# huggingface/tokenizers

Hardware: AMD Instinct MI355X
Metric: GB input text/sec (whole node), GPT-2 BPE encode_batch (higher is better)
Workload: dtype u8->u32

## Files before the change

tokenizers_amd/csrc/capi/api_handle.cpp:

```cpp

#pragma GCC visibility push(default)
extern "C" {

const char* tkamd_version(void) { return "tokenizers_amd 0.1.0 (gfx950)"; }
const char* tkamd_last_error(void) { return g_last_error.c_str(); }

static std::unique_ptr<tkamd_tokenizer> make_tokenizer(const char* json, size_t json_len, int device, const tkamd_tokenizer* primary) {
    std::unique_ptr<tkamd_tokenizer> t(new tkamd_tokenizer());
    if (primary) { t->hm = primary->hm; t->n_direct = primary->n_direct; }
    else t->hm = HostModel::from_json(json, json_len);
    t->device = device;
    if (device >= 0) {
        check_not_forked();
        int n = 0;
        if (hipGetDeviceCount(&n) != hipSuccess || n == 0) throw HipError("no HIP device available (the HIP path has no CPU fallback)");
        if (device >= n) throw HipError("HIP device ordinal out of range");
        HIP_CHECK(hipSetDevice(device));
        note_hip_used();
        hipDeviceProp_t prop;
        HIP_CHECK(hipGetDeviceProperties(&prop, device));
        t->n_cu = prop.multiProcessorCount > 0 ? prop.multiProcessorCount : 256;
        if (const char* e = test_hook("TKAMD_Q16_DIV")) t->q16_div = (uint32_t)std::max(1, atoi(e));
        upload_tables(t.get());
        if (prepare_long_kernel() != 0) throw HipError("hipFuncSetAttribute(dynamic LDS) failed");
        if (!primary) verify_direct_words(t.get());
        build_shortw_table(t.get());
        build_hot_table(t.get());
        if (const char* e = test_hook("TKAMD_CLAIMS_PAUSE")) t->claims_pause_len = std::max(0, atoi(e));
        if (const char* e = test_hook("TKAMD_ADDED_SPEC")) t->added_spec_len = std::max(0, atoi(e));
        if (const char* e = test_hook("TKAMD_NFC_SPEC")) t->nfc_spec_len = std::max(0, atoi(e));
        t->cp_grid = compact_grid(t->n_cu);
        if (const char* e = test_hook("TKAMD_CP_GRID")) t->cp_grid = std::max(1, atoi(e));
        t->devices.push_back(device);
    }
    return t;
}

static std::vector<int> devices_from_env() {
    std::vector<int> d;
    const char* e = getenv("TOKENIZERS_GPU_DEVICES");
    if (!e || !*e) return {0};
    if (!strcmp(e, "all")) {
        int n = 0;
        if (hipGetDeviceCount(&n) != hipSuccess || n == 0) throw HipError("no HIP device available (the HIP path has no CPU fallback)");
        for (int i = 0; i < n; ++i) d.push_back(i);
        return d;
    }
    for (const char* q = e; *q;) {
        char* end = nullptr;
        const long v = strtol(q, &end, 10);
        if (end == q || v < 0 || v > 1023) throw Invalid("TOKENIZERS_GPU_DEVICES: expected \"all\" or a comma-separated list of device ordinals");
        d.push_back((int)v);
        q = end;
        if (*q == ',') ++q;
        else if (*q) throw Invalid("TOKENIZERS_GPU_DEVICES: expected \"all\" or a comma-separated list of device ordinals");
    }
    if (d.empty()) d.push_back(0);
    return d;
}

int tkamd_tokenizer_from_json(const char* json, size_t json_len, int device, tkamd_tokenizer** out) {
    if (!json || !out) return set_error(TKAMD_ERR_INVALID, "null argument");
    *out = nullptr;
    return guarded([&]() -> int {
        *out = make_tokenizer(json, json_len, device, nullptr).release();
        return TKAMD_OK;
    });
}

int tkamd_tokenizer_from_json_devices(const char* json, size_t json_len, const int* devices, int n_devices, tkamd_tokenizer** out) {
    if (!json || !out || n_devices < 0 || (n_devices > 0 && !devices)) return set_error(TKAMD_ERR_INVALID, "bad argument");
    *out = nullptr;
    return guarded([&]() -> int {
        std::vector<int> devs = n_devices ? std::vector<int>(devices, devices + n_devices) : devices_from_env();
        if (devs.size() > 64) throw Invalid("more than 64 devices");
        for (int d : devs) if (d < 0) throw Invalid("a multi-device handle needs device ordinals >= 0");
        std::unique_ptr<tkamd_tokenizer> t = make_tokenizer(json, json_len, devs[0], nullptr);
        for (size_t r = 1; r < devs.size(); ++r) {
            t->replicas.push_back(make_tokenizer(nullptr, 0, devs[r], t.get()));
            if (devs[r] != devs[0]) {
                const hipError_t e = hipDeviceEnablePeerAccess(devs[0], 0);
                if (e != hipSuccess) (void)hipGetLastError();
            }
        }
        t->devices = devs;
        if (const char* e = getenv("TKAMD_SHARD_MIN_KB")) t->shard_min_bytes = (int64_t)std::max(1, atoi(e)) << 10;
        HIP_CHECK(hipSetDevice(devs[0]));
        *out = t.release();
        return TKAMD_OK;
    });
}

int tkamd_tokenizer_set_collect(tkamd_tokenizer* t, int mode) {
    if (!t || mode < TKAMD_COLLECT_HOST || mode > TKAMD_COLLECT_ROOT_RCCL) return set_error(TKAMD_ERR_INVALID, "bad argument");
    if (mode == TKAMD_COLLECT_ROOT_RCCL && !test_hook("TKAMD_RCCL_LIB")) {
        std::vector<int> seen;
        for (int d : t->devices) {
            if (std::find(seen.begin(), seen.end(), d) != seen.end()) return set_error(TKAMD_ERR_INVALID, "TKAMD_COLLECT_ROOT_RCCL: a device is named twice (RCCL wants one rank per GPU)");
            seen.push_back(d);
        }
    }
    t->collect = mode;
    return TKAMD_OK;
}

int tkamd_tokenizer_devices(const tkamd_tokenizer* t, int* devices, int cap, int* n) {
    if (!t || !n) return set_error(TKAMD_ERR_INVALID, "null argument");
    *n = (int)t->devices.size();
    for (int i = 0; i < *n && i < cap && devices; ++i) devices[i] = t->devices[(size_t)i];
    return TKAMD_OK;
}

int tkamd_shard_stats(const tkamd_tokenizer* t, int64_t* shard_bytes, double* busy_ms, int cap, int* n) {
    if (!t || !n) return set_error(TKAMD_ERR_INVALID, "null argument");
    std::lock_guard<std::mutex> lk(const_cast<tkamd_tokenizer*>(t)->group_mu);
    *n = (int)t->shard_ms.size();
    for (int i = 0; i < *n && i < cap; ++i) {
        if (shard_bytes) shard_bytes[i] = t->shard_bytes[(size_t)i];
        if (busy_ms) busy_ms[i] = t->shard_ms[(size_t)i];
    }
    return TKAMD_OK;
}

void tkamd_tokenizer_free(tkamd_tokenizer* t) {
    if (!t) return;
    if (g_forked) {
        for (auto& r : t->replicas) (void)r.release();
        return;
    }
    for (void* c : t->rccl_comms) if (c) rccl_api().CommDestroy(c);
    t->rccl_comms.clear();
    for (auto& r : t->replicas) tkamd_tokenizer_free(r.release());
    t->replicas.clear();
    if (t->device >= 0) {
        (void)hipSetDevice(t->device);
        (void)hipDeviceSynchronize();
        std::lock_guard<std::mutex> lk(t->mu);
        for (auto& w : t->pool) drain_profile(t, w.get());
    }
    delete t;
}

int tkamd_tokenizer_info(const tkamd_tokenizer* t, tkamd_info* info) {
    if (!t || !info) return set_error(TKAMD_ERR_INVALID, "null argument");
    const HostModel& hm = t->hm;
    info->model = (int32_t)hm.model;
    info->pre_tokenizer = (int32_t)hm.pretok;
    info->normalizer = (int32_t)(hm.nfc_lower ? NORM_NFC_LOWER : hm.norm);
    info->vocab_size = (int32_t)hm.vocab_size;
    info->n_merges = (int32_t)hm.n_merges;
    info->add_prefix_space = hm.add_prefix_space;
    info->ignore_merges = hm.ignore_merges;
    info->n_added_tokens = (int32_t)hm.added_tokens.size();
    info->device = t->device;
    info->n_direct_words = t->n_direct;
    info->truncation = hm.trunc_on ? (int32_t)hm.trunc_max_length : -1;
    info->padding = !hm.pad_on ? 0 : (hm.pad_left ? 2 : 1);
    info->pad_id = (int32_t)hm.pad_id;
    info->pad_type_id = (int32_t)hm.pad_type_id;
    info->word_disp_entries = 0;
    info->merge_disp_entries = (int32_t)hm.merge_disp.size();
    return TKAMD_OK;
}

int tkamd_tokenizer_specials(const tkamd_tokenizer* t, uint32_t* prefix_ids, int32_t* n_prefix, uint32_t* suffix_ids, int32_t* n_suffix,
                             int32_t cap) {
    if (!t || !n_prefix || !n_suffix) return set_error(TKAMD_ERR_INVALID, "null argument");
    if (!t->hm.pp_unsupported.empty()) return set_error(TKAMD_ERR_UNSUPPORTED, "add_special_tokens: " + t->hm.pp_unsupported);
    *n_prefix = (int32_t)t->hm.pp_prefix.size();
    *n_suffix = (int32_t)t->hm.pp_suffix.size();
    for (int32_t i = 0; i < *n_prefix && i < cap && prefix_ids; ++i) prefix_ids[i] = t->hm.pp_prefix[i];
    for (int32_t i = 0; i < *n_suffix && i < cap && suffix_ids; ++i) suffix_ids[i] = t->hm.pp_suffix[i];
    return TKAMD_OK;
}

int tkamd_tokenizer_pair_template(const tkamd_tokenizer* t, int with_specials, uint32_t* pieces, int32_t cap, int32_t* n_pieces) {
    if (!t || !n_pieces) return set_error(TKAMD_ERR_INVALID, "null argument");
    if (with_specials && !t->hm.pp_pair_unsupported.empty()) return set_error(TKAMD_ERR_UNSUPPORTED, "add_special_tokens on a pair: " + t->hm.pp_pair_unsupported);
    const std::vector<HostModel::TplPiece>& tpl = (with_specials && !t->hm.pp_pair.empty()) ? t->hm.pp_pair : t->hm.pp_pair_plain;
    *n_pieces = (int32_t)tpl.size();
    for (int32_t i = 0; i < *n_pieces && i < cap && pieces; ++i) { pieces[3 * i] = tpl[i].kind; pieces[3 * i + 1] = tpl[i].id; pieces[3 * i + 2] = tpl[i].type_id; }
    return TKAMD_OK;
}

static int encode_device(tkamd_tokenizer* t, const uint8_t* d_text, const int64_t* d_doc_offsets, int64_t n_docs, int64_t n_bytes,
// ... 37 lines not shown
```

tokenizers_amd/csrc/capi/handle.cpp:

```cpp

struct Workspace {
    std::mutex mu;
    std::function<uint32_t(uint32_t)> pad_exchange;
    uint32_t h_padmax = 0;
    bool busy = false;
    bool device_bound = false;
    hipStream_t bound_stream = nullptr;
    hipStream_t own_stream = nullptr;
    hipStream_t io_in = nullptr, io_out = nullptr;
    hipEvent_t ev_in[2] = {nullptr, nullptr}, ev_out[2] = {nullptr, nullptr};
    DevBuf w_l3_tiles;
    DevBuf w_ptext, w_pnorig, w_pdoc_off, w_pc_ltot;
    DevBuf w_ms_dmask, w_pprefix, w_pt_word;
    DevBuf w_docmask, w_startmask, w_wprefix, w_bsum, w_tile_w, w_pt_start, w_tok0, w_pt_tokoff, w_tmp_ids, w_tmp_end, w_rows;
    DevBuf w_len1, w_fin, w_fbsum, w_pad_count, w_keep, w_type_ids2, w_seq_ids2;
    DevBuf w_ovf_parts, w_enc_base, w_enc_doc, w_enc_start, w_enc_cnt;
    DevBuf w_enc_idx, w_enc_win;
    DevBuf w_queues, w_qcount, w_cstate;
    DevBuf w_doc_off;
    DevBuf w_chunk_lo;
    DevBuf w_ids, w_doc_pt, w_tok_offsets, w_scalars, w_offsets, w_word_ids;
    DevBuf dw_ids, dw_tok_off, dw_first, dw_bad, dw_dup, dw_len, dw_bsum, dw_pos, dw_out_off, dw_bytes, dw_total;
    DevBuf w_endmask, w_pt_end, w_keepmask, w_kprefix, w_ntext, w_norig, w_ndoc_off, w_slow_docs, w_leadmask, w_lprefix, w_need, w_need_bsum, w_huge, w_list_huge, w_wbase, w_norig_e, w_ids2, w_tok_offsets2, w_offsets2, w_word_ids2, w_candmask, w_matchmask, w_spanmask, w_stopmask, w_hardmask, w_boundmask, w_bprefix, w_seg_off, w_xseg_off,
        w_match_docs, w_match_list;
    DevBuf h_text, h_doc_off, h_seq_off, h_inp_off;
    DevBuf w_uni_state, w_uni_flags;
    DevBuf w_tok_b8;
    DevBuf w_trim1;
    const uint8_t* cur_trim1 = nullptr;
    DevBuf w_cache_keys, w_cache_rows;
    DevBuf w_claims, w_claim_rows, w_claim_pos;
    DevBuf w_phases;
    uint64_t cache_epoch = 0;
    DevBuf w_seq_off, w_seq_tok_off, w_word_idx, w_first_tok;
    std::vector<StageRec> pending;
    const uint8_t* last_text = nullptr;
    const int64_t* last_doc_off = nullptr;
    const int64_t* last_seq_off = nullptr;
    int64_t last_n_seqs = -1;
    const int64_t* last_inp_off = nullptr;
    int64_t last_n_inputs = -1;
    DevBuf w_inp_off;
    DevBuf w_mask_dirty;
    int64_t last_n_bytes = 0;
    uint32_t last_flags = 0;
    tkamd_device_result last_result{};
    int64_t last_n_docs = 0;
    int64_t last_n_enc = -1;
    int last_ntok_slot = 1;
    uint32_t last_counters[CNT_COUNT] = {0};
    bool force_general = false;
    bool force_nfc = false;
    bool last_note_nfc = false;
    bool last_note_added = false;
    bool last_used_claims = false;
    ~Workspace() {
        if (own_stream) (void)hipStreamDestroy(own_stream);
        if (io_in) (void)hipStreamDestroy(io_in);
        if (io_out) (void)hipStreamDestroy(io_out);
        for (int i = 0; i < 2; ++i) {
            if (ev_in[i]) (void)hipEventDestroy(ev_in[i]);
            if (ev_out[i]) (void)hipEventDestroy(ev_out[i]);
        }
    }
};

struct tkamd_tokenizer {
    HostModel hm;
    int device = -1;
    DevTables dt{};
    std::mutex mu;
    std::condition_variable cv;
    std::vector<std::unique_ptr<Workspace>> pool;
    Workspace* last_used = nullptr;
    DevBuf t_ucc1, t_ucc2;
    DevBuf t_uc1, t_uc2, t_byte_id, t_merges, t_long_blob, t_long_off, t_long_id, t_long_table;
    DevBuf t_hot;
    DevBuf t_shortw, t_shortw_k3, t_shortw_disp;
    DevBuf t_char_id;
    DevBuf t_at_id[2], t_at_flags[2], t_at_blob[2], t_at_off[2], t_at_first[2];
    DevBuf t_pp_single, t_pp_single_plain;
    DevBuf t_pp_pair, t_pp_pair_plain;
    DevBuf t_pp_prefix, t_pp_suffix, t_pp_prefix_ty, t_pp_suffix_ty, t_bn1, t_bn2, t_bn_map, t_nfc1, t_nfc2, t_nfc_map, t_nfk_map, t_nfk_flat, t_pc_units, t_pc_rep, t_gc1, t_gc2, t_merge_disp, t_dec_entry, t_dec_blob, t_trie, t_uni_score, t_uni_is_byte;
    int n_cu = 256;
    int n_direct = 0;
    int n_hot = 0;
    uint32_t shortw_max_disp = 0;
    int cp_grid = 0;
    std::atomic<int> claims_pause{0};
    std::atomic<int> added_spec_pause{0};
    std::atomic<int> nfc_spec_pause{0};
    std::atomic<uint32_t> nfc_reruns{0};
    int nfc_spec_len = 32;
    int added_spec_len = 32;
    int claims_pause_len = 32;
    std::atomic<uint32_t> q16_div{4};
    std::atomic<bool> prof{false};
    std::atomic<bool> encode_special{false};
    std::atomic<bool> word_cache{false};
    std::atomic<uint64_t> cache_epoch{1};
    std::vector<tkamd_stage_time> acc;
    std::vector<int> devices;
    std::vector<std::unique_ptr<tkamd_tokenizer>> replicas;
    std::mutex group_mu;
    std::atomic<int> collect{0};
    std::string collect_note;
    std::vector<std::unique_ptr<DevBuf>> g_root;
    std::vector<void*> rccl_comms;
    int64_t shard_min_bytes = 1 << 20;
    std::vector<double> shard_ms;
    std::vector<int64_t> shard_bytes;
};

constexpr size_t PHASE_WGS = 1 << 17;
constexpr size_t MAX_HOST_WORKSPACES = 4;

struct PinnedBlock {
    void* p = nullptr;
    size_t cap = 0;
};
static std::mutex g_pin_mu;
static std::vector<PinnedBlock> g_pin_free;

static PinnedBlock pinned_get(size_t bytes) {
    if (bytes < 64) bytes = 64;
    {
        std::lock_guard<std::mutex> lk(g_pin_mu);
        size_t best = (size_t)-1;
        for (size_t i = 0; i < g_pin_free.size(); ++i)
            if (g_pin_free[i].cap >= bytes && (best == (size_t)-1 || g_pin_free[i].cap < g_pin_free[best].cap)) best = i;
        if (best != (size_t)-1 && g_pin_free[best].cap <= 2 * bytes + (1u << 20)) {
            PinnedBlock b = g_pin_free[best];
            g_pin_free.erase(g_pin_free.begin() + best);
            return b;
        }
    }
    PinnedBlock b;
    size_t want = bytes + bytes / 8;
    HIP_CHECK(hipHostMalloc(&b.p, want, hipHostMallocPortable));
    b.cap = want;
    return b;
}
static void pinned_put(PinnedBlock b) {
    if (!b.p || g_forked) return;
    std::lock_guard<std::mutex> lk(g_pin_mu);
    if (g_pin_free.size() >= 16) { (void)hipHostFree(b.p); return; }
    g_pin_free.push_back(b);
}

struct tkamd_batch {
    int64_t n_docs = 0, n_tokens = 0;
    PinnedBlock ids, tok_offsets, offsets, word_ids, pad_counts, type_ids, seq_ids, enc_docs, enc_parts;
    bool has_offsets = false, has_words = false, has_pads = false, has_types = false, has_enc_docs = false, has_enc_parts = false;
    ~tkamd_batch() { pinned_put(ids); pinned_put(tok_offsets); pinned_put(offsets); pinned_put(word_ids); pinned_put(pad_counts); pinned_put(type_ids); pinned_put(seq_ids); pinned_put(enc_docs); pinned_put(enc_parts); }
};

struct tkamd_text {
    int64_t n_docs = 0, n_bytes = 0;
    PinnedBlock bytes, doc_offsets;
    ~tkamd_text() { pinned_put(bytes); pinned_put(doc_offsets); }
};
```

tokenizers_amd/csrc/capi/pipeline.cpp:

```cpp

int lookup_grid(const tkamd_tokenizer* t) { return std::min(3 * t->n_cu, (int)NSQ); }

struct QueueSizes {
    uint32_t sq_cap[4], row_base[4];
    size_t total;
};
static bool rerun_wanted(tkamd_tokenizer* t, Workspace* w, int raw) {
    const int err = raw & ~NOTE_BITS;
    bool again = false;
    if (raw & NOTE_ADDED_SEEN) { t->added_spec_pause = t->added_spec_len; w->force_general = true; again = true; }
    if (raw & NOTE_NFC_SEEN) { t->nfc_spec_pause = t->nfc_spec_len; w->force_nfc = true; ++t->nfc_reruns; again = true; }
    if (err == ERR_QUEUE_FULL && t->q16_div > 1) { t->q16_div = t->q16_div > 2 ? 2 : 1; again = true; }
    return again;
}

QueueSizes queue_sizes(size_t N, uint32_t q16_div, int grid) {
    QueueSizes z{};
    const size_t n_tiles = N / LOOKUP_TILE_BYTES + 1;
    const size_t per_sq = ((n_tiles + grid - 1) / grid) * LOOKUP_TILE_BYTES;
    z.sq_cap[0] = (uint32_t)(per_sq / q16_div + 64);
    z.sq_cap[1] = (uint32_t)(per_sq / 17 + 16);
    z.sq_cap[2] = (uint32_t)(per_sq / 33 + 16);
    z.sq_cap[3] = (uint32_t)(per_sq / 65 + 16);
    size_t acc = 0;
// ... 596 lines not shown
        }
        pf.begin("pretok_llama3");
        w->w_slow_docs.reserve((size_t)((piece_off ? seg_cap : (size_t)n_docs) + 1) * 4);
        launch_pretok_llama3(st, x_text, n_x, x_len_dev, w->w_docmask.as<ull>(), t->dt.uc1, t->dt.uc2, w->w_startmask.as<ull>(),
                             w->w_endmask.as<ull>(), piece_off ? piece_off : x_doc_off, piece_off ? (int64_t)seg_cap : n_docs, piece_n_dev,
                             w->w_slow_docs.as<uint32_t>(), d_counters + CNT_SLOW_DOCS, hm.split_rule,
                             t->t_ucc1.p ? t->t_ucc1.as<uint16_t>() : nullptr, t->t_ucc2.p ? t->t_ucc2.as<uint8_t>() : nullptr,
                             w->w_l3_tiles.p ? w->w_l3_tiles.as<ull>() : nullptr, lead_done ? w->w_leadmask.as<ull>() : nullptr);
        pf.end();
    } else if (hm.pretok == PT_SPLIT_CHAIN) {
        w->w_endmask.reserve((size_t)(W + 1) * 8);
        if (off_mode == TKAMD_OFFSETS_CHAR && x_text == d_text && !x_len_dev && n_x == n_bytes) {
            w->w_leadmask.reserve((size_t)(W0 + 1) * 8);
            lead_done = true;
        }
        pf.begin("pretok_ds3");
        w->w_slow_docs.reserve((size_t)((piece_off ? seg_cap : (size_t)n_docs) + 1) * 4);
        launch_pretok_ds3(st, x_text, n_x, x_len_dev, w->w_docmask.as<ull>(), t->dt.uc1, t->dt.uc2, t->t_ucc1.as<uint16_t>(), t->t_ucc2.as<uint8_t>(),
                          w->w_startmask.as<ull>(), w->w_endmask.as<ull>(), piece_off ? piece_off : x_doc_off, piece_off ? (int64_t)seg_cap : n_docs, piece_n_dev,
                          w->w_slow_docs.as<uint32_t>(), d_counters + CNT_SLOW_DOCS, lead_done ? w->w_leadmask.as<ull>() : nullptr);
        pf.end();
    } else if (hm.pretok == PT_DIGITS_GPT2) {
        if (off_mode == TKAMD_OFFSETS_CHAR && x_text == d_text && !x_len_dev && n_x == n_bytes) {
            w->w_leadmask.reserve((size_t)(W0 + 1) * 8);
            lead_done = true;
        }
        pf.begin("pretok_digits");
        launch_pretok_digits(st, x_text, n_x, x_len_dev, w->w_docmask.as<ull>(), t->dt.uc1, t->dt.uc2, hm.digits_individual, w->w_startmask.as<ull>(),
                             lead_done ? w->w_leadmask.as<ull>() : nullptr);
        pf.end();
    } else if (hm.pretok == PT_CLIP) {
        w->w_endmask.reserve((size_t)(W + 1) * 8);
        has_end = true;
        if (off_mode == TKAMD_OFFSETS_CHAR && x_text == d_text && !x_len_dev && n_x == n_bytes) {
            w->w_leadmask.reserve((size_t)(W0 + 1) * 8);
            lead_done = true;
        }
        pf.begin("pretok_clip");
        launch_pretok_clip(st, x_text, n_x, x_len_dev, w->w_docmask.as<ull>(), t->dt.uc1, t->dt.uc2, w->w_startmask.as<ull>(), w->w_endmask.as<ull>(),
                           lead_done ? w->w_leadmask.as<ull>() : nullptr);
        pf.end();
    } else if (metaspace) {
        pf.begin("metaspace_units");
        launch_ms_units(st, x_text, n_x, x_len_dev, w->w_docmask.as<ull>(), w->w_startmask.as<ull>(), W, hm.ms_split);
        pf.end();
    } else if (hm.pretok == PT_BYTELEVEL_NOREGEX) {
        HIP_CHECK(hipMemcpyAsync(w->w_startmask.p, w->w_docmask.p, (size_t)W * 8, hipMemcpyDeviceToDevice, st));
    } else {
        w->w_endmask.reserve((size_t)(W + 1) * 8);
        has_end = true;
        if (want_meta) {
            w->w_pt_end.reserve(((size_t)n_x + 4) * 4);
            pt_end = w->w_pt_end.as<uint32_t>();
        }
        pf.begin("pretok_local");
        launch_pretok_local(st, (int)hm.pretok, x_text, n_x, x_len_dev, w->w_docmask.as<ull>(), t->dt.uc1, t->dt.uc2,
                            w->w_startmask.as<ull>(), w->w_endmask.as<ull>(), true);
        pf.end();
    }
    if (matchmask)
        launch_apply_matches(st, w->w_startmask.as<ull>(), has_end ? w->w_endmask.as<ull>() : nullptr, matchmask, w->w_spanmask.as<ull>(),
                             w->w_stopmask.as<ull>(), W, n_match);
    pf.begin("mask_scan");
    meta_masks = want_meta && !(hm.char_bpe && !hm.unk_configured && !hm.byte_fallback);
    if (meta_masks) w->w_tile_w.reserve(((size_t)n_x / META_TILE + 4) * 4);
    launch_mask_scan(st, w->w_startmask.as<ull>(), W, w->w_bsum.as<uint32_t>(), w->w_wprefix.as<uint32_t>(), d_npretok, x_len_dev,
                     meta_masks ? w->w_tile_w.as<uint32_t>() : nullptr);
    pf.end();
    if (want_meta && !meta_masks) {
        pf.begin("emit_pretok");
        launch_emit_pretok(st, w->w_startmask.as<ull>(), w->w_wprefix.as<uint32_t>(), n_x, x_len_dev, d_npretok, w->w_pt_start.as<uint32_t>());
        if (pt_end) launch_emit_pretok_end(st, w->w_startmask.as<ull>(), w->w_endmask.as<ull>(), w->w_wprefix.as<uint32_t>(), n_x, x_len_dev, pt_end);
        pf.end();
    }
    pf.begin("doc_first_pretok");
    launch_doc_first_pretok(st, lean ? raw_doc_off : x_doc_off, n_docs, n_x, w->w_startmask.as<ull>(), w->w_wprefix.as<uint32_t>(),
                            d_npretok, w->w_doc_pt.as<uint32_t>(), w->w_chunk_lo.as<uint32_t>(),
                            lean ? d_err : nullptr, lean ? w->w_doc_off.as<int64_t>() : nullptr);
    pf.end();
    if (metaspace && !hm.ms_split && want_words && !words_in) {
        w->w_pprefix.reserve((size_t)(W + 2) * 4);
        w->w_pt_word.reserve(((size_t)n_x + 4) * 4);
        pf.begin("metaspace_words");
        launch_mask_scan(st, w->w_docmask.as<ull>(), W, w->w_bsum.as<uint32_t>(), w->w_pprefix.as<uint32_t>(), sc + SC_NPIECE, x_len_dev);
        launch_ms_piece_rank(st, w->w_startmask.as<ull>(), w->w_wprefix.as<uint32_t>(), w->w_docmask.as<ull>(), w->w_pprefix.as<uint32_t>(), n_x, x_len_dev,
                             w->w_pt_word.as<uint32_t>());
        pf.end();
        pt_word = w->w_pt_word.as<uint32_t>();
    }
}

void* Batch::phases_of(int which) {
    if (!test_hook("TKAMD_PHASES")) return nullptr;
    if (!w->w_phases.p) {
        w->w_phases.reserve(2 * PHASE_WGS * 64);
        HIP_CHECK(hipMemsetAsync(w->w_phases.p, 0, 2 * PHASE_WGS * 64, st));
    }
    return (uint8_t*)w->w_phases.p + (size_t)which * PHASE_WGS * 64;
}

void Batch::open_word_cache() {
    const size_t slots = (size_t)1 << WORD_CACHE_BITS;
    if (use_claims) {
        uint32_t* cpos = nullptr;
        if (off_mode != TKAMD_OFFSETS_NONE) { w->w_claim_pos.reserve(claim_slots * 4); cpos = w->w_claim_pos.as<uint32_t>(); }
        wc = WordCache{nullptr, w->w_claim_rows.p, (unsigned long long*)w->w_claims.p, (uint32_t)(claim_slots - 1), cpos};
        return;
    }
    if (!t->word_cache || off_mode != TKAMD_OFFSETS_NONE) return;
    w->w_cache_keys.reserve(slots * sizeof(CacheKey));
    w->w_cache_rows.reserve(slots * 16);
    const uint64_t epoch = t->cache_epoch;
    if (w->cache_epoch != epoch) {
        HIP_CHECK(hipMemsetAsync(w->w_cache_keys.p, 0, slots * sizeof(CacheKey), st));
        w->cache_epoch = epoch;
    }
    wc = WordCache{(CacheKey*)w->w_cache_keys.p, w->w_cache_rows.p, nullptr, 0u, nullptr};
}

void Batch::run_model() {
    tmp_end = (off_mode != TKAMD_OFFSETS_NONE) ? w->w_tmp_end.as<uint32_t>() : nullptr;
    const size_t N = (size_t)n_x;
    const QueueSizes qz = queue_sizes(N, t->q16_div, lookup_grid(t));
    static const size_t row_limit = [] { const char* e = test_hook("TKAMD_ROW_LIMIT_BITS"); return e ? std::min<size_t>((size_t)1 << std::max(8, atoi(e)), ROW_INDEX_LIMIT) : (size_t)ROW_INDEX_LIMIT; }();
    if (qz.total >= row_limit) throw Invalid("batch too large for the work queues (row indices are 30-bit: about 3 GB of text): split it");
    QueuePlan plan{};
    for (int c = 0; c < 4; ++c) {
        plan.v[c].q = (QItem*)(w->w_queues.as<uint8_t>() + (size_t)qz.row_base[c] * 8);
        plan.v[c].counts = w->w_qcount.as<uint32_t>() + (size_t)c * NSQ * QCNT_STRIDE;
        plan.v[c].sq_cap = qz.sq_cap[c];
        plan.v[c].row_base = qz.row_base[c];
    }
    const ull* endmask = has_end ? w->w_endmask.as<ull>() : nullptr;
    DevTables mdt = t->dt;
    mdt.err = d_err;
    mdt.probes = t->prof ? d_counters + CNT_MERGE_PROBES : nullptr;
    auto set_publish = [&]() {
        if (wc.claims) { mdt.pub_rows = wc.rows; mdt.pub_mask = wc.claim_mask; mdt.pub_pos = wc.claim_pos; }
    };
    if (hm.model == MODEL_BPE) {
        pf.begin("lookup");
        open_word_cache();
        set_publish();
        launch_lookup(st, lookup_grid(t), t->dt, x_text, n_x, x_len_dev, w->w_startmask.as<ull>(), endmask, w->w_wprefix.as<uint32_t>(),
                      w->w_tok0.as<uint32_t>(), plan, d_err, matchmask, t->t_hot.p, wc, 0u, 0u, phases_of(0), d_counters);
        pf.end();
        if (hm.ignore_merges)
            launch_long_vocab3(st, t->n_cu, t->dt, x_text, plan.v[1], plan.v[2], plan.v[3], w->w_rows.p, 0u, d_err, wc);
        const bool lds = t->dt.newid_affine && !test_hook("TKAMD_FORCE_LANE_MERGE");
        const bool can_one = wc.claims && lds && !test_hook("TKAMD_MERGE_TWO");
        const char* const pair_hook = test_hook("TKAMD_MERGE_PAIR");
        const bool pair = can_one && !(pair_hook && pair_hook[0] == '0');
        const bool one = can_one && !pair;
        const size_t huge_words = std::min<size_t>((size_t)6 * N + 4096, (size_t)1 << 28);
        const bool huge_possible = N > (size_t)LONG_PT_MAX;
        if (huge_possible) {
            w->w_huge.reserve(huge_words * 4);
            w->w_list_huge.reserve((N / LONG_PT_MAX + 16) * 4);
        } else {
            w->w_huge.reserve(64);
            w->w_list_huge.reserve(64);
        }
        auto long_tail = [&]() {
            launch_bpe_merge_long(st, t->n_cu, mdt, x_text, plan.v[3], w->w_rows.p, w->w_tmp_ids.as<uint32_t>(), tmp_end, w->w_list_huge.as<uint32_t>(),
                                  d_counters + CNT_LISTH, w->w_huge.as<uint32_t>(), (unsigned long long)(huge_possible ? huge_words : 0),
                                  (unsigned long long*)(sc + SC_HUGE_USED), d_err);
        };
        if (hm.char_bpe) {
            auto long_only = [&](const QView& q) {
                launch_bpe_merge_long_only(st, t->n_cu * 2, mdt, x_text, q, w->w_rows.p, w->w_tmp_ids.as<uint32_t>(), tmp_end, w->w_list_huge.as<uint32_t>(), d_counters + CNT_LISTH);
            };
            pf.begin("bpe_merge_lds32");
            if (t->dt.newid_affine) launch_bpe_merge(st, t->n_cu, 6, mdt, x_text, plan.v[1], w->w_rows.p, w->w_tmp_ids.as<uint32_t>(), tmp_end, nullptr);
            else long_only(plan.v[1]);
            pf.end();
            pf.begin("bpe_merge_lds");
            if (t->dt.newid_affine) launch_bpe_merge(st, t->n_cu, 5, mdt, x_text, plan.v[0], w->w_rows.p, w->w_tmp_ids.as<uint32_t>(), tmp_end);
            else long_only(plan.v[0]);
            pf.end();
            pf.begin("bpe_merge_long");
            long_only(plan.v[2]);
            long_tail();
            pf.end();
        } else {
            if (pair) {
                pf.begin("bpe_merge_lds_pair");
                launch_bpe_merge_pair(st, t->n_cu, mdt, x_text, plan.v[0], plan.v[1], w->w_rows.p, w->w_tmp_ids.as<uint32_t>(), tmp_end);
                pf.end();
            } else {
                pf.begin(lds ? "bpe_merge_lds32" : "bpe_merge_lane32");
                launch_bpe_merge(st, lds ? t->n_cu : grid, lds ? 6 : 2, mdt, x_text, plan.v[1], w->w_rows.p, w->w_tmp_ids.as<uint32_t>(), tmp_end, one ? &plan.v[0] : nullptr);
                pf.end();
            }
            if (!can_one) {
                pf.begin(lds ? "bpe_merge_lds" : "bpe_merge_lane");
                launch_bpe_merge(st, lds ? t->n_cu : grid, lds ? 5 : 1, mdt, x_text, plan.v[0], w->w_rows.p, w->w_tmp_ids.as<uint32_t>(), tmp_end);
                pf.end();
            }
            pf.begin("bpe_merge64");
            launch_bpe_merge(st, grid, 64, mdt, x_text, plan.v[2], w->w_rows.p, w->w_tmp_ids.as<uint32_t>(), tmp_end);
            pf.end();
            pf.begin("bpe_merge_long");
            long_tail();
            pf.end();
        }
        if (wc.keys) {
            pf.begin("word_cache_insert");
            launch_word_cache_insert(st, grid, mdt, x_text, plan.v[0], w->w_rows.p, wc);
            pf.end();
        }
    } else if (hm.model == MODEL_UNIGRAM) {
        if (use_claims) open_word_cache();
        set_publish();
        pf.begin("lookup");
        launch_lookup(st, lookup_grid(t), t->dt, x_text, n_x, x_len_dev, w->w_startmask.as<ull>(), endmask, w->w_wprefix.as<uint32_t>(),
                      w->w_tok0.as<uint32_t>(), plan, d_err, matchmask, t->t_hot.p, wc, 0u, 0u, phases_of(0), d_counters);
        pf.end();
        w->w_uni_state.reserve(N > 64 ? (N + 2) * 16 : 64);
        pf.begin("unigram");
        launch_unigram_all(st, grid, t->n_cu, mdt, x_text, plan, w->w_rows.p, w->w_tmp_ids.as<uint32_t>(), tmp_end, d_err, w->w_uni_state.p);
        pf.end();
    } else if (hm.model == MODEL_WORDLEVEL) {
        DevTables wt = t->dt;
        wt.ignore_merges = 1;
        pf.begin("wordlevel_lookup");
        launch_lookup(st, lookup_grid(t), wt, x_text, n_x, x_len_dev, w->w_startmask.as<ull>(), endmask, w->w_wprefix.as<uint32_t>(),
                      w->w_tok0.as<uint32_t>(), plan, d_err, matchmask, t->t_hot.p, WordCache{nullptr, nullptr, nullptr, 0u, nullptr}, 0u, 1u, nullptr, nullptr);
        launch_long_vocab3(st, t->n_cu, wt, x_text, plan.v[1], plan.v[2], plan.v[3], w->w_rows.p, 1u, d_err, WordCache{nullptr, nullptr, nullptr, 0u, nullptr});
        pf.end();
    } else {
        const bool shortcut = hm.max_input_chars >= (uint32_t)WORD_MAX_KEY;
        DevTables wt = t->dt;
        wt.ignore_merges = 1;
        wt.long_probe_max_len = hm.max_input_chars;
        if (shortcut) open_word_cache();
        set_publish();
        pf.begin("wordpiece_word_lookup");
        launch_lookup(st, lookup_grid(t), wt, x_text, n_x, x_len_dev, w->w_startmask.as<ull>(), endmask, w->w_wprefix.as<uint32_t>(),
                      w->w_tok0.as<uint32_t>(), plan, d_err, matchmask, t->t_hot.p, wc, shortcut ? 0u : 1u, 0u, phases_of(0), d_counters);
        pf.end();
        pf.begin("wordpiece");
        launch_wordpiece_all(st, grid, t->n_cu, mdt, x_text, plan, w->w_rows.p, w->w_tmp_ids.as<uint32_t>(), tmp_end, d_err);
        pf.end();
        if (wc.keys) {
            pf.begin("word_cache_insert");
            launch_word_cache_insert(st, grid, t->dt, x_text, plan.v[0], w->w_rows.p, wc);
            pf.end();
        }
    }
    if (matchmask)
        launch_apply_match_ids(st, w->w_match_list.as<uint32_t>(), d_counters + CNT_MATCHES, w->w_startmask.as<ull>(),
                               w->w_wprefix.as<uint32_t>(), w->w_tok0.as<uint32_t>());
}

void Batch::compact_and_meta() {
    uint8_t* tok_b8 = nullptr;
    if (tmp_end) { w->w_tok_b8.reserve((size_t)n_x + 64); tok_b8 = w->w_tok_b8.as<uint8_t>(); }
    pf.begin("compact");
    launch_compact(st, t->cp_grid, w->w_tok0.as<uint32_t>(), w->w_rows.p, wc.rows, w->w_tmp_ids.as<uint32_t>(), d_npretok, w->w_cstate.as<ull>(),
                   d_ntok_total, want_meta ? w->w_pt_tokoff.as<uint32_t>() : nullptr, w->w_ids.as<uint32_t>(), w->w_chunk_lo.as<uint32_t>(),
                   w->w_doc_pt.as<uint32_t>(), n_docs, w->w_tok_offsets.as<int64_t>(), (size_t)t->cp_grid <= PHASE_WGS ? phases_of(1) : nullptr, tok_b8);
    pf.end();
    const uint32_t* word_of_doc = nullptr;
    const int64_t* first_tok = nullptr;
    if (words_in) {
        if (want_words) { w->w_word_idx.reserve((size_t)(n_docs + 2) * 4); word_of_doc = w->w_word_idx.as<uint32_t>(); }
        if (off_mode != TKAMD_OFFSETS_NONE && hm.trim_offsets) { w->w_first_tok.reserve((size_t)(n_docs + 2) * 8); first_tok = w->w_first_tok.as<int64_t>(); }
        launch_seq_regroup(st, d_seq_off, n_seqs, n_docs, w->w_tok_offsets.as<int64_t>(), w->w_seq_tok_off.as<int64_t>(), (uint32_t*)word_of_doc, (int64_t*)first_tok);
    }
    if (want_meta) {
        MetaArgs a{};
        a.word_of_doc = word_of_doc;
        a.pt_word = pt_word;
        a.first_tok = first_tok;
        a.x_text = x_text;
        a.text = d_text;
        a.pt_start = meta_masks ? nullptr : w->w_pt_start.as<uint32_t>();
        a.pt_end = meta_masks ? nullptr : pt_end;
        a.startmask = w->w_startmask.as<ull>();
        a.endmask = has_end ? w->w_endmask.as<ull>() : nullptr;
        a.wprefix = w->w_wprefix.as<uint32_t>();
        a.tile_w = meta_masks ? w->w_tile_w.as<uint32_t>() : nullptr;
        a.n_mask_words = W;
        a.x_len_dev = x_len_dev;
        a.x_len_host = n_x;
        a.n_tok = d_ntok_total;
        a.pt_tokoff = w->w_pt_tokoff.as<uint32_t>();
        a.tmp_end = tmp_end;
        a.tok_b8 = tok_b8;
        a.tok0 = wc.claims ? w->w_tok0.as<uint32_t>() : nullptr;
        a.claim_pos = wc.claims ? wc.claim_pos : nullptr;
        a.n_pretok = d_npretok;
        a.doc_pt = w->w_doc_pt.as<uint32_t>();
        a.chunk_lo = w->w_chunk_lo.as<uint32_t>();
        a.chunk = (uint32_t)COMPACT_CHUNK;
        a.n_docs = n_docs;
        a.x_doc_off = x_doc_off;
        a.doc_off = d_doc_off;
        a.norig = norig;
        a.norig_e = norig_e;
        a.byte_level = hm.byte_level;
        a.snap_chars = hm.byte_level || hm.char_bpe || hm.uni_bytes;
        if (hm.char_bpe && !hm.unk_configured && !hm.byte_fallback) {
            a.char_id = t->dt.char_id;
            a.cb = t->dt.cb;
            if (hm.ignore_merges) { a.ww_tok0 = w->w_tok0.as<uint32_t>(); a.ww_rows = w->w_rows.p; a.ww_crows = wc.rows; }
        }
        a.trim_offsets = hm.trim_offsets;
        a.trim_matches_only = !hm.byte_level;
        a.pp_add_prefix_space = hm.pp_add_prefix_space;
        a.want_offsets = off_mode != TKAMD_OFFSETS_NONE;
        a.char_mode = off_mode == TKAMD_OFFSETS_CHAR;
        a.want_words = want_words;
        a.matchmask = matchmask;
        a.uc1 = t->dt.uc1;
        a.uc2 = t->dt.uc2;
        a.offsets = w->w_offsets.as<uint32_t>();
        a.word_ids = w->w_word_ids.as<uint32_t>();
        if (a.want_offsets && a.trim_offsets && a.pp_add_prefix_space && hm.trunc_on) {
            w->w_trim1.reserve((size_t)n_x + 8);
            a.trim1 = w->w_trim1.as<uint8_t>();
            w->cur_trim1 = a.trim1;
        }
        if (a.char_mode) {
            w->w_leadmask.reserve((size_t)(W0 + 1) * 8);
            w->w_lprefix.reserve((size_t)(W0 + 1) * 4);
            pf.begin("leadmask_scan");
            if (!lead_done) launch_leadmask(st, d_text, n_bytes, w->w_leadmask.as<ull>());
            launch_mask_scan(st, w->w_leadmask.as<ull>(), W0, w->w_bsum.as<uint32_t>(), w->w_lprefix.as<uint32_t>(), sc + SC_NCHARS);
            pf.end();
            a.leadmask = w->w_leadmask.as<ull>();
            a.lprefix = w->w_lprefix.as<uint32_t>();
        }
        pf.begin("token_meta");
        launch_token_meta(st, grid, a);
        pf.end();
        if (a.want_offsets && hm.uni_bytes) {
            w->w_uni_flags.reserve((size_t)n_x + 64);
            pf.begin("unigram_run_offsets");
            launch_unigram_run_offsets(st, grid, t->dt, w->w_ids.as<uint32_t>(), a.offsets, w->w_tok_offsets.as<int64_t>(), n_docs, d_ntok_total, w->w_uni_flags.as<uint8_t>());
// ... 108 lines not shown
```

tokenizers_amd/csrc/capi/probes.cpp:

```cpp

int tkamd_probe_word(const tkamd_tokenizer* t, const uint8_t* bytes, int32_t len, uint32_t* id, uint32_t* flags) {
    if (!t || !bytes || !id || !flags || len < 0) return set_error(TKAMD_ERR_INVALID, "bad argument");
    const HostModel& hm = t->hm;
    *id = 0;
    *flags = 0;
    if (len == 0 || hm.word_table.empty()) return 0;
    if (len <= WORD_MAX_KEY) {
        uint8_t buf[16] = {0};
        memcpy(buf, bytes, (size_t)len);
        uint64_t lo, hi;
        memcpy(&lo, buf, 8);
        memcpy(&hi, buf + 8, 8);
        const uint32_t h1 = word_hash1(lo, hi, (uint32_t)len, hm.word_seed);
        const WordSlot& sa = hm.word_table[word_slot_a(h1, hm.word_mask)];
        const WordSlot& s = (sa.len == (uint32_t)len && sa.lo == lo && sa.hi == hi) ? sa : hm.word_table[word_slot_b(h1, hm.word_mask)];
        if (s.len != (uint32_t)len || s.lo != lo || s.hi != hi) return 0;
        *id = s.id;
        *flags = s.flags;
        return 1;
    }
    if (hm.long_table.empty()) return 0;
    uint32_t h = fnv1a(bytes, (size_t)len) & hm.long_mask;
    for (;;) {
        const uint32_t e = hm.long_table[h];
// ... 69 lines not shown
    if (!o.empty()) { memcpy(out, o.data(), o.size()); memcpy(src, al.data(), al.size() * 4); }
    return TKAMD_OK;
}

int tkamd_probe_norm_chain(const tkamd_tokenizer* t, const uint8_t* text, int64_t n, uint8_t* out, uint32_t* src, int64_t cap, int64_t* n_out) {
    if (!t || (!text && n) || n < 0 || !n_out || cap < 0 || (cap && (!out || !src))) return set_error(TKAMD_ERR_INVALID, "bad argument");
    const HostModel& hm = t->hm;
    if (hm.norm != NORM_CHAIN) return set_error(TKAMD_ERR_UNSUPPORTED, "the tokenizer has no NFD / Lowercase / StripAccents normalizer");
    std::vector<uint32_t> al;
    bool refused = false;
    const std::string o = hm.chain_normalize(std::string((const char*)text, (size_t)n), &al, &refused);
    if (refused) return set_error(TKAMD_ERR_UNSUPPORTED, "NFD: a character is followed by more than 48 combining characters; the normalization of such a run is not built");
    *n_out = (int64_t)o.size();
    if ((int64_t)o.size() > cap) return set_error(TKAMD_ERR_INVALID, "the output buffer is too small");
    if (!o.empty()) { memcpy(out, o.data(), o.size()); memcpy(src, al.data(), al.size() * 4); }
    return TKAMD_OK;
}

int tkamd_probe_nfkc(const tkamd_tokenizer* t, const uint8_t* text, int64_t n, uint8_t* out, uint32_t* src, int64_t cap, int64_t* n_out) {
    if (!t || (!text && n) || n < 0 || !n_out || cap < 0 || (cap && (!out || !src))) return set_error(TKAMD_ERR_INVALID, "bad argument");
    const HostModel& hm = t->hm;
    if (hm.norm != NORM_NFKC) return set_error(TKAMD_ERR_UNSUPPORTED, "the tokenizer has no NFKC normalizer");
    std::vector<uint32_t> al;
    bool refused = false;
    const std::string o = hm.nfkc_normalize(std::string((const char*)text, (size_t)n), &al, &refused);
    if (refused) return set_error(TKAMD_ERR_UNSUPPORTED, "NFKC: a character is followed by more than 48 combining characters; the normalization of such a run is not built");
    *n_out = (int64_t)o.size();
    if ((int64_t)o.size() > cap) return set_error(TKAMD_ERR_INVALID, "the output buffer is too small");
    if (!o.empty()) { memcpy(out, o.data(), o.size()); memcpy(src, al.data(), al.size() * 4); }
    return TKAMD_OK;
}

int tkamd_probe_bert_alone(const tkamd_tokenizer* t, const uint8_t* text, int64_t n, int64_t pos, int32_t* reorder, int32_t* alone) {
    if (!t || !text || !reorder || !alone || n < 0 || pos < 0 || pos >= n) return set_error(TKAMD_ERR_INVALID, "bad argument");
    const HostModel& hm = t->hm;
    if (hm.norm != NORM_BERT) return set_error(TKAMD_ERR_UNSUPPORTED, "the tokenizer has no BertNormalizer");
    uint32_t len;
    const uint32_t cp = bn_core_decode(text, pos, n, &len);
    const uint32_t f = bn_core_flags(hm.bn_stage1.data(), hm.bn_stage2.data(), cp);
    *reorder = (hm.bn_strip_accents && (f & BN_F_REORDER)) ? 1 : 0;
    *alone = (!*reorder || bn_alone_in_run(hm.bn_stage1.data(), hm.bn_stage2.data(), hm.bn_clean_text, text, 0, n, pos, len, f, nullptr)) ? 1 : 0;
    return TKAMD_OK;
}

int tkamd_probe_bert_nfd(const tkamd_tokenizer* t, uint32_t cp, uint32_t* packed, uint32_t* flags) {
    if (!t || !packed || !flags) return set_error(TKAMD_ERR_INVALID, "null argument");
    const HostModel& hm = t->hm;
    if (hm.norm != NORM_BERT) return set_error(TKAMD_ERR_UNSUPPORTED, "the tokenizer has no BertNormalizer");
    const BnCoreTables ct{hm.bn_stage1.data(), hm.bn_stage2.data(), hm.bn_map.data(), hm.bn_mask, hm.bn_seed, hm.bn_clean_text};
    uint32_t lo = 0, hi = 0;
    *packed = bn_core_map(ct, cp, 2u, &lo, &hi) ? lo : 0u;
    *flags = bn_core_flags(ct.bn1, ct.bn2, cp);
    return TKAMD_OK;
}

int64_t tkamd_text_n_docs(const tkamd_text* b) { return b ? b->n_docs : 0; }
int64_t tkamd_text_n_bytes(const tkamd_text* b) { return b ? b->n_bytes : 0; }
const uint8_t* tkamd_text_bytes(const tkamd_text* b) { return b ? (const uint8_t*)b->bytes.p : nullptr; }
const int64_t* tkamd_text_doc_offsets(const tkamd_text* b) { return b ? (const int64_t*)b->doc_offsets.p : nullptr; }
void tkamd_text_free(tkamd_text* b) { delete b; }

int tkamd_encode_special_tokens(tkamd_tokenizer* t, int value) {
    if (!t) return set_error(TKAMD_ERR_INVALID, "null argument");
    t->encode_special = value != 0;
    for (auto& r : t->replicas) r->encode_special = value != 0;
    return TKAMD_OK;
}

int tkamd_word_cache(tkamd_tokenizer* t, int enable, int clear) {
    if (!t) return set_error(TKAMD_ERR_INVALID, "null argument");
    if (clear) ++t->cache_epoch;
    t->word_cache = enable != 0;
    for (auto& r : t->replicas) { if (clear) ++r->cache_epoch; r->word_cache = enable != 0; }
    return TKAMD_OK;
}

int tkamd_profile_enable(tkamd_tokenizer* t, int on) {
    if (!t) return set_error(TKAMD_ERR_INVALID, "null argument");
    t->prof = on != 0;
    for (auto& r : t->replicas) r->prof = on != 0;
    return TKAMD_OK;
}

int tkamd_profile_read(tkamd_tokenizer* t, tkamd_stage_time* stages, int max_stages, int* n_stages, int reset) {
    if (!t || !n_stages) return set_error(TKAMD_ERR_INVALID, "null argument");
    std::lock_guard<std::mutex> lk(t->mu);
    if (t->device >= 0 && !g_forked) {
        (void)hipSetDevice(t->device);
        for (auto& w : t->pool) drain_profile(t, w.get());
        for (auto& r : t->replicas) {
            std::lock_guard<std::mutex> rl(r->mu);
            (void)hipSetDevice(r->device);
            for (auto& w : r->pool) drain_profile(t, w.get());
        }
        if (!t->replicas.empty()) (void)hipSetDevice(t->device);
    }
    int n = (int)std::min<size_t>(t->acc.size(), (size_t)std::max(0, max_stages));
    for (int i = 0; i < n && stages; ++i) stages[i] = t->acc[i];
    *n_stages = n;
    if (reset) t->acc.clear();
    return TKAMD_OK;
}

int tkamd_pinned_alloc(size_t bytes, void** out) {
    if (!out) return set_error(TKAMD_ERR_INVALID, "null argument");
    *out = nullptr;
    return guarded([&]() -> int {
        check_not_forked();
        void* p = nullptr;
        note_hip_used();
        HIP_CHECK(hipHostMalloc(&p, bytes ? bytes : 64, hipHostMallocPortable));
        *out = p;
        return TKAMD_OK;
    });
}
void tkamd_pinned_free(void* p) {
    if (p && !g_forked) (void)hipHostFree(p);
}

int tkamd_debug_phases(tkamd_tokenizer* t, int which, uint64_t* out, int reset) {
    if (!t || !out || which < 0 || which > 1) return set_error(TKAMD_ERR_INVALID, "bad argument");
    return guarded([&]() -> int {
        for (int k = 0; k < 8; ++k) out[k] = 0;
        if (t->device < 0 || g_forked) return TKAMD_OK;
        HIP_CHECK(hipSetDevice(t->device));
        HIP_CHECK(hipDeviceSynchronize());
        std::lock_guard<std::mutex> lk(t->mu);
        std::vector<uint64_t> h(PHASE_WGS * 8);
        for (auto& w : t->pool) {
            if (!w->w_phases.p) continue;
            uint8_t* const p = (uint8_t*)w->w_phases.p + (size_t)which * PHASE_WGS * 64;
            HIP_CHECK(hipMemcpy(h.data(), p, PHASE_WGS * 64, hipMemcpyDeviceToHost));
            for (size_t g = 0; g < PHASE_WGS; ++g)
                for (int k = 0; k < 8; ++k) out[k] += h[g * 8 + k];
            if (reset) HIP_CHECK(hipMemset(p, 0, PHASE_WGS * 64));
        }
        return TKAMD_OK;
    });
}

int tkamd_profile_counters(tkamd_tokenizer* t, uint32_t* out, int n) {
    if (!t || !out) return set_error(TKAMD_ERR_INVALID, "null argument");
    return guarded([&]() -> int {
        std::lock_guard<std::mutex> lk(t->mu);
        Workspace* w = t->last_used;
        for (int i = 0; i < n; ++i) out[i] = 0;
        if (n > 18) out[18] = t->dt.shortw ? t->dt.shortw_mask + 1u : 0u;
        if (n > 19) out[19] = t->dt.shortw ? t->dt.shortw_bmask + 1u : 0u;
        if (n > 20) out[20] = t->shortw_max_disp;
        if (n > 21) out[21] = (uint32_t)t->hm.merge_table.size();
        if (!w) return TKAMD_OK;
        for (int i = 0; i < n && i < CNT_COUNT; ++i) out[i] = w->last_counters[i];
        if (n > 13) out[13] = (uint32_t)pair_merge_occupancy();
        if (n > 14) out[14] = (uint32_t)std::max(0, t->added_spec_pause.load());
        if (n > 15) out[15] = t->q16_div;
        if (n > 16) out[16] = (uint32_t)std::max(0, t->nfc_spec_pause.load());
        if (n > 17) out[17] = t->nfc_reruns.load();
        if (t->device >= 0 && w->w_qcount.p && !g_forked) {
            HIP_CHECK(hipSetDevice(t->device));
            HIP_CHECK(hipDeviceSynchronize());
            std::vector<uint32_t> c(QCNT_WORDS);
            HIP_CHECK(hipMemcpy(c.data(), w->w_qcount.p, (size_t)QCNT_WORDS * 4, hipMemcpyDeviceToHost));
            static const int slot[4] = {CNT_LIST16, CNT_LIST32, CNT_LIST64, CNT_LISTL};
            for (int q = 0; q < 4; ++q) {
                uint32_t sum = 0;
                for (int i = 0; i < NSQ; ++i) sum += c[((size_t)q * NSQ + i) * QCNT_STRIDE];
                if (slot[q] < n) out[slot[q]] = sum;
            }
        }
        return TKAMD_OK;
    });
}

}
#pragma GCC visibility pop
```

tokenizers_amd/csrc/kernels.hip:

```cpp
#include <hip/hip_runtime.h>
#include <cstdlib>
#include <cstring>

#include <algorithm>
#include <cstdint>

#include "device_utils.hpp"
#include "kernels.hpp"
#include "overflow_core.hpp"
#include "bert_norm_core.hpp"
#include "nfc_core.hpp"
#include "precompiled_core.hpp"
#include "pretok_gpt2_core.hpp"
#include "pretok_l3_core.hpp"
#include "pretok_ds3_core.hpp"
#include "pretok_digits_core.hpp"
#include "pretok_clip_core.hpp"
#include "pretok_local_core.hpp"
#include "unigram_core.hpp"
#include "tables.hpp"

namespace tkamd {

__device__ __forceinline__ uint32_t uc_flags(uint32_t cp, const uint16_t* __restrict__ uc1, const uint8_t* __restrict__ uc2) {
    if (cp >= 0x110000u) return 0;
    return uc2[((uint32_t)uc1[cp >> 8] << 8) | (cp & 255u)];
}

struct __attribute__((packed, aligned(1))) Unaligned4 { uint32_t v; };
struct __attribute__((packed, aligned(1))) Unaligned16 { uint32_t a, b, c, d; };
#if defined(__HIP_DEVICE_COMPILE__)
typedef uint32_t nt_u32x4 __attribute__((ext_vector_type(4), aligned(1)));
__device__ __forceinline__ Unaligned16 load_nt16(const uint8_t* p) { const nt_u32x4 v = __builtin_nontemporal_load((const nt_u32x4*)p); return Unaligned16{v.x, v.y, v.z, v.w}; }
template <class T> __device__ __forceinline__ T load_nt(const T* p) { return __builtin_nontemporal_load(p); }
template <class T> __device__ __forceinline__ void store_nt(T* p, T v) { __builtin_nontemporal_store(v, p); }
typedef uint32_t nt_a_u32x4 __attribute__((ext_vector_type(4)));
typedef uint32_t nt_a_u32x2 __attribute__((ext_vector_type(2)));
__device__ __forceinline__ uint4 load_nt(const uint4* p) { const nt_a_u32x4 v = __builtin_nontemporal_load((const nt_a_u32x4*)p); return make_uint4(v.x, v.y, v.z, v.w); }
__device__ __forceinline__ uint2 load_nt(const uint2* p) { const nt_a_u32x2 v = __builtin_nontemporal_load((const nt_a_u32x2*)p); return make_uint2(v.x, v.y); }
__device__ __forceinline__ void store_nt(uint2* p, uint2 v) { nt_a_u32x2 x; x.x = v.x; x.y = v.y; __builtin_nontemporal_store(x, (nt_a_u32x2*)p); }
#else
__device__ __forceinline__ Unaligned16 load_nt16(const uint8_t* p) { return *(const Unaligned16*)p; }
template <class T> __device__ __forceinline__ T load_nt(const T* p) { return *p; }
template <class T> __device__ __forceinline__ void store_nt(T* p, T v) { *p = v; }
#endif
__device__ __forceinline__ uint32_t utf8_global(const uint8_t* __restrict__ text, int64_t i, uint32_t* len) {
    uint32_t w = ((const Unaligned4*)(text + i))->v;
    uint32_t b0 = w & 0xFFu, b1 = (w >> 8) & 0x3Fu, b2 = (w >> 16) & 0x3Fu, b3 = (w >> 24) & 0x3Fu;
    if (b0 < 0x80u) { *len = 1; return b0; }
    if (b0 < 0xE0u) { *len = 2; return ((b0 & 0x1Fu) << 6) | b1; }
    if (b0 < 0xF0u) { *len = 3; return ((b0 & 0x0Fu) << 12) | (b1 << 6) | b2; }
    *len = 4;
    return ((b0 & 0x07u) << 18) | (b1 << 12) | (b2 << 6) | b3;
}
static inline unsigned blocks_for(int64_t n, int per_block) { return (unsigned)((n + per_block - 1) / per_block); }

#include "kernels/results.hip"
#include "kernels/scan_util.hip"
#include "kernels/documents.hip"
#include "kernels/pretok_gpt2.hip"
#include "kernels/pretok_llama3.hip"
#include "kernels/pretok_ds3.hip"
#include "kernels/pretok_digits.hip"
#include "kernels/pretok_clip.hip"
#include "kernels/pretok_local.hip"
#include "kernels/bert_norm.hip"
#include "kernels/nfc.hip"
#include "kernels/precompiled.hip"
#include "kernels/nfkc.hip"
#include "kernels/metaspace.hip"
#include "kernels/scan_emit.hip"
#include "kernels/bpe.hip"
#include "kernels/lookup.hip"
#include "kernels/word_models.hip"
#include "kernels/unigram.hip"
#include "kernels/bpe_huge.hip"
#include "kernels/output.hip"
#include "kernels/epilogue.hip"
#include "kernels/decode.hip"
#include "kernels/launch.hip"

}
```

tokenizers_amd/csrc/kernels.hpp:

```cpp
#pragma once
#include <hip/hip_runtime_api.h>
#include <cstdint>

#include "nfc_core.hpp"
#include "precompiled_core.hpp"
#include "tables.hpp"

namespace tkamd {

struct DevTables {
    const uint16_t* uc1;
    const uint8_t* uc2;
    const uint32_t* byte_id;
    const uint32_t* byte_sfx;
    const MergeSlot* merges;
    const uint16_t* merge_disp;
    uint32_t merge_mask, merge_seed, merge_bmask;
    uint32_t newid_affine, newid_base;
    const uint32_t* char_id;
    uint32_t cb;
    int* err;
    uint32_t* probes;
    void* pub_rows;
    uint32_t* pub_pos;
// ... 123 lines not shown
    const uint32_t* first;
    const uint32_t* id;
    const uint32_t* flags;
    unsigned long long first_set[4];
    uint32_t n_first;
    uint32_t first_byte[4];
    uint32_t skip_special;
};

struct SpecialArgs {
    const int64_t* tok_offsets;
    int64_t n_docs;
    const uint32_t* ids;
    const uint32_t* offsets;
    const uint32_t* word_ids;
    const uint32_t* prefix;
    const uint32_t* suffix;
    int32_t n_prefix, n_suffix;
    int64_t* tok_offsets2;
    uint32_t* ids2;
    uint32_t* offsets2;
    uint32_t* word_ids2;
    int64_t* n_tok2;
};

struct FinalArgs {
    const int64_t* tok_offsets;
    int64_t n_docs;
    const uint32_t* ids;
    const uint32_t* offsets;
    const uint32_t* word_ids;
    const uint8_t* trim1;
    const uint32_t* prefix;
    const uint32_t* suffix;
    int32_t n_prefix, n_suffix;
    uint32_t trunc_len;
    uint32_t trunc_left;
    uint32_t trunc_needs_pair;
    uint32_t trunc_stride;
    uint32_t pad_on, pad_fixed, pad_length, pad_multiple, pad_left, pad_id;
    uint32_t* ovf_parts;
    int64_t* enc_base;
    uint32_t* enc_doc;
    uint32_t* enc_start;
    uint32_t* enc_cnt;
    uint32_t* len1;
    uint32_t* fin;
    uint32_t* target;
    uint32_t* bsum;
    int64_t* tok_offsets2;
    uint32_t* ids2;
    uint32_t* offsets2;
    uint32_t* word_ids2;
    uint32_t* pad_count;
    int64_t* n_tok2;
    int* err;
    uint8_t* type_ids2;
    uint8_t* seq_ids2;
    const uint8_t* prefix_ty;
    const uint8_t* suffix_ty;
    uint32_t seq_ty;
    uint32_t pad_type_id;
};

struct PairArgs {
    const int64_t* tok_offsets;
    int64_t n_pairs;
    const uint32_t* ids;
    const uint32_t* offsets;
    const uint32_t* word_ids;
    const uint8_t* trim1;
    const uint32_t* tpl;
    int32_t n_tpl;
    uint32_t n_special;
    const int64_t* inp_off;
    const uint32_t* tpl1;
    int32_t n_tpl1;
    uint32_t n_special1;
    uint32_t trunc_on, trunc_max, trunc_left, trunc_strategy, trunc_stride;
    uint32_t pad_on, pad_fixed, pad_length, pad_multiple, pad_left, pad_id, pad_type_id;
    uint32_t* keep;
    uint32_t first_is_b;
    uint32_t ovf_ty_tpl;
    uint32_t* ovf_parts;
    int64_t* enc_base;
    uint32_t* enc_doc;
    uint32_t* enc_idx;
    uint32_t* enc_win;
    uint32_t* len1;
    uint32_t* fin;
    uint32_t* target;
    uint32_t* bsum;
    int64_t* tok_offsets2;
    uint32_t* ids2;
    uint32_t* offsets2;
    uint32_t* word_ids2;
    uint8_t* type_ids2;
    uint8_t* seq_ids2;
    uint32_t* pad_count;
    int64_t* n_tok2;
    int* err;
};

enum : int {
    ERR_BAD_OFFSETS = 1,
    ERR_PRETOKEN_TOO_LONG = 2,
    ERR_ADDED_SPLIT = 4,
    ERR_NON_ASCII_NORM = 8,
    ERR_MISSING_UNK = 16,
    ERR_INTERNAL = 32,
    ERR_QUEUE_FULL = 64,
    ERR_TRUNC_SECOND = 128,
    ERR_TOO_MANY_TOKENS = 256,
    ERR_TRUNC_SHORT = 512,
    ERR_TRUNC_STRIDE = 1024,
    ERR_INPUT_KIND = 8192,
    ERR_UNK_OOV = 4096,
    NOTE_REORDER_SEEN = 2048,
    NOTE_ADDED_SEEN = 16384,
    NOTE_NFC_SEEN = 32768,
    ERR_NFC_SEGMENT = 65536,
    NOTE_PC_LOST = 131072,
    NOTE_BITS = NOTE_REORDER_SEEN | NOTE_ADDED_SEEN | NOTE_NFC_SEEN | NOTE_PC_LOST,
    ERR_QUEUE_FULL_PAD = 0,
};

enum : int { CNT_LIST16 = 0, CNT_LIST64 = 1, CNT_LISTL = 2, CNT_LIST32 = 3, CNT_SLOW_DOCS = 4, CNT_CLAIM_CANDS = 5, CNT_CLAIM_SHARED = 6, CNT_LISTH = 7, CNT_MATCH_DOCS = 8,
              CNT_MATCHES = 9, CNT_MATCH_DOCS2 = 10, CNT_CLAIM_GAVE_UP = 11, CNT_MERGE_PROBES = 12, CNT_COUNT = 13 };

constexpr uint32_t MATCH_LEN_ORIG = 0x80000000u;
constexpr int TEXT_PAD = 64;
constexpr int LONG_PT_MAX = 8192;

void launch_mark_doc_starts(hipStream_t st, const int64_t* doc_off, int64_t n_docs, int64_t n_bytes,
                            unsigned long long* docmask, int* err);
void launch_validate_csr(hipStream_t st, const int64_t* doc_off, int64_t n_docs, int64_t n_bytes, int* err, int64_t* san);
void launch_pretok_gpt2(hipStream_t st, const uint8_t* text, int64_t n_bytes, const int64_t* len_dev, const unsigned long long* docmask,
                        const uint16_t* uc1, const uint8_t* uc2, unsigned long long* startmask, unsigned long long* leadmask = nullptr);
void launch_mask_scan(hipStream_t st, const unsigned long long* mask, int64_t n_words, uint32_t* bsum, uint32_t* wprefix,
                      int64_t* total, const int64_t* len_dev = nullptr, uint32_t* tile_w = nullptr);
void launch_emit_pretok(hipStream_t st, const unsigned long long* startmask, const uint32_t* wprefix, int64_t n_bytes,
                        const int64_t* len_dev, const int64_t* n_pretok, uint32_t* pt_start);
void launch_prefix_space(hipStream_t st, const uint8_t* text, const int64_t* seg_off, int64_t n_bound, const int64_t* n_dev, const unsigned long long* matchmask,
                         uint32_t* need, uint32_t* bsum, int64_t* xseg_off, int64_t* x_len, uint8_t* xtext, uint32_t* nos, uint32_t* noe, int grid);
void launch_doc_first_pretok(hipStream_t st, const int64_t* doc_off, int64_t n_docs, int64_t n_bytes,
                             const unsigned long long* startmask, const uint32_t* wprefix, const int64_t* n_pretok, uint32_t* doc_pt, uint32_t* chunk_lo,
                             const int* err = nullptr, int64_t* san = nullptr);
void launch_lookup(hipStream_t st, int grid, const DevTables& t, const uint8_t* text, int64_t n_bytes, const int64_t* len_dev,
                   const unsigned long long* startmask, const unsigned long long* endmask, const uint32_t* wprefix, uint32_t* tok0,
                   const QueuePlan& plan, int* err, const unsigned long long* matchmask, const void* hot, const WordCache& wc,
                   uint32_t no_hits, uint32_t miss_is_unk, void* phases = nullptr, uint32_t* counters = nullptr);
void launch_bpe_merge(hipStream_t st, int grid, int group, const DevTables& t, const uint8_t* text, const QView& v, void* rows,
                      uint32_t* tmp_ids, uint32_t* tmp_end, const QView* also = nullptr);
void launch_bpe_merge_pair(hipStream_t st, int n_cu, const DevTables& t, const uint8_t* text, const QView& v16, const QView& v32, void* rows,
                           uint32_t* tmp_ids, uint32_t* tmp_end);
int pair_merge_occupancy();
inline size_t bn_olen_bytes(int64_t n_bytes) { return (((size_t)n_bytes + 64 + 15) & ~(size_t)15) + ((size_t)n_bytes >> 4) + 64; }
inline uint8_t* bn_ltot_of(uint8_t* olen, int64_t n_bytes) { return olen + (((size_t)n_bytes + 64 + 15) & ~(size_t)15); }
void launch_mark_doc_starts_n(hipStream_t st, const int64_t* doc_off, int64_t n_docs, int64_t n_bytes, const int64_t* len_dev,
                              unsigned long long* docmask, int* err);
void launch_pretok_local(hipStream_t st, int kind, const uint8_t* text, int64_t n_bytes, const int64_t* len_dev, const unsigned long long* docmask,
                         const uint16_t* uc1, const uint8_t* uc2, unsigned long long* startmask, unsigned long long* endmask, bool len_bound = false);
void launch_emit_pretok_end(hipStream_t st, const unsigned long long* startmask, const unsigned long long* endmask,
                            const uint32_t* wprefix, int64_t n_bytes, const int64_t* len_dev, uint32_t* pt_end);
void launch_bert_normalize(hipStream_t st, const BnTables& bt, const uint8_t* text, int64_t n_bytes, const int64_t* doc_off, int64_t n_docs,
                           const unsigned long long* verbatim, uint8_t* olen, uint32_t* wsum, uint32_t* bsum, uint32_t* wbase, int64_t* x_len, uint8_t* ntext,
                           uint32_t* nos, uint32_t* noe, int64_t* ndoc_off, int* err);
void launch_nfc_check(hipStream_t st, const NfcTables& nt, const uint8_t* text, int64_t n_bytes, int* note);
void launch_nfc_bound(hipStream_t st, unsigned long long* dmask, const unsigned long long* verbatim, int64_t n_words);
void launch_nfc_normalize(hipStream_t st, const NfcTables& nt, const uint8_t* text, int64_t n_bytes, const int64_t* doc_off, int64_t n_docs,
                          const unsigned long long* verbatim, const unsigned long long* bound, uint8_t* olen, uint32_t* wsum, uint32_t* bsum, uint32_t* wbase,
                          int64_t* x_len, uint8_t* ntext, uint32_t* nos, int64_t* ndoc_off, int* err);
void launch_long_vocab3(hipStream_t st, int grid, const DevTables& t, const uint8_t* text, const QView& v1, const QView& v2, const QView& v3, void* rows, uint32_t miss_is_unk,
                        int* err, const WordCache& wc);
void launch_unigram_all(hipStream_t st, int grid_short, int grid_long, const DevTables& t, const uint8_t* text, const QueuePlan& plan, void* rows, uint32_t* tmp_ids,
                        uint32_t* tmp_end, int* err, void* state);
void launch_unigram_run_offsets(hipStream_t st, int grid, const DevTables& t, const uint32_t* ids, uint32_t* offsets, const int64_t* tok_offsets, int64_t n_docs,
                                const int64_t* n_tok, uint8_t* flags);
void launch_wordpiece_all(hipStream_t st, int grid_short, int grid_long, const DevTables& t, const uint8_t* text, const QueuePlan& plan, void* rows, uint32_t* tmp_ids,
                          uint32_t* tmp_end, int* err);
void launch_pretok_llama3(hipStream_t st, const uint8_t* text, int64_t n_bytes, const int64_t* len_dev, const unsigned long long* docmask,
                          const uint16_t* uc1, const uint8_t* uc2, unsigned long long* startmask, unsigned long long* slowmask,
                          const int64_t* doc_off, int64_t n_docs, const int64_t* n_docs_dev, uint32_t* slow_docs, uint32_t* n_slow_docs,
                          SplitRule rule, const uint16_t* ucc1, const uint8_t* ucc2, unsigned long long* tileflags, unsigned long long* leadmask = nullptr);
inline size_t l3_tileflag_words(int64_t n_bytes) { return (size_t)((n_bytes + 1) / 2048 + 1) / 64 + 2; }
void launch_pretok_ds3(hipStream_t st, const uint8_t* text, int64_t n_bytes, const int64_t* len_dev, const unsigned long long* docmask,
                       const uint16_t* uc1, const uint8_t* uc2, const uint16_t* ps1, const uint8_t* ps2, unsigned long long* startmask, unsigned long long* slowmask,
                       const int64_t* doc_off, int64_t n_docs, const int64_t* n_docs_dev, uint32_t* slow_docs, uint32_t* n_slow_docs, unsigned long long* leadmask = nullptr);
void launch_pretok_digits(hipStream_t st, const uint8_t* text, int64_t n_bytes, const int64_t* len_dev, const unsigned long long* docmask,
                          const uint16_t* uc1, const uint8_t* uc2, bool individual, unsigned long long* startmask, unsigned long long* leadmask = nullptr);
void launch_pretok_clip(hipStream_t st, const uint8_t* text, int64_t n_bytes, const int64_t* len_dev, const unsigned long long* docmask,
                        const uint16_t* uc1, const uint8_t* uc2, unsigned long long* startmask, unsigned long long* endmask, unsigned long long* leadmask = nullptr);
void launch_leadmask(hipStream_t st, const uint8_t* text, int64_t n_bytes, unsigned long long* leadmask);
void launch_seq_regroup(hipStream_t st, const int64_t* seq_off, int64_t n_seqs, int64_t n_words, const int64_t* word_tok_off, int64_t* seq_tok_off, uint32_t* widx,
                        int64_t* first_tok);
void launch_token_meta(hipStream_t st, int grid, const MetaArgs& a);
void launch_add_specials(hipStream_t st, int grid, const SpecialArgs& a);
void launch_add_i64(hipStream_t st, int64_t* data, int64_t n, int64_t delta);
void launch_add_u32(hipStream_t st, uint32_t* data, int64_t n, uint32_t delta);
void launch_final_lens(hipStream_t st, const FinalArgs& a);
void launch_overflow_count(hipStream_t st, const FinalArgs& a, int64_t* n_enc);
void launch_overflow_ranges(hipStream_t st, const FinalArgs& a);
void launch_final_offsets(hipStream_t st, const FinalArgs& a);
void launch_finalize(hipStream_t st, int grid, const FinalArgs& a);
void launch_pair_lens(hipStream_t st, const PairArgs& a);
void launch_pair_overflow_scan(hipStream_t st, const PairArgs& a, int64_t* n_enc);
void launch_pair_ranges(hipStream_t st, const PairArgs& a);
void launch_pair_finalize(hipStream_t st, int grid, const PairArgs& a);
void launch_added_match(hipStream_t st, const AddedArgs& a, const uint8_t* text, int64_t n_bytes, const int64_t* len_dev, const int64_t* seg_off, int64_t n_segs,
                        const int64_t* n_segs_dev, const unsigned long long* skipmask, const uint16_t* uc1, const uint8_t* uc2, unsigned long long* candmask,
                        uint32_t* sents, uint32_t* n_sents, uint32_t* match_list, uint32_t* n_match, uint32_t cap, uint32_t len_flag, int* err);
void launch_added_detect(hipStream_t st, const AddedArgs& a, const uint8_t* text, int64_t n_bytes, const int64_t* len_dev, int* note);
void launch_scatter_matches(hipStream_t st, const uint32_t* list, const uint32_t* n_list, int64_t n_bytes, const int64_t* len_dev, unsigned long long* matchmask,
                            unsigned long long* spanmask, unsigned long long* stopmask, unsigned long long* hardmask, uint32_t* tmp_end, uint32_t* dirty);
void launch_mask_or2(hipStream_t st, unsigned long long* dst, const unsigned long long* a, const unsigned long long* b, int64_t n_words);
void launch_emit_boundaries(hipStream_t st, const unsigned long long* mask, const uint32_t* wprefix, int64_t n_bytes, const int64_t* len_dev, const int64_t* total, int64_t* out);
void launch_metaspace(hipStream_t st, const uint8_t* text, int64_t n_bytes, const int64_t* doc_off, int64_t n_docs, const unsigned long long* pstart,
                      const unsigned long long* dstart, const unsigned long long* mmask, const unsigned long long* smask, uint32_t prepend, uint8_t* olen,
                      uint32_t* wsum, uint32_t* bsum, uint32_t* wbase, int64_t* x_len, uint8_t* xtext, uint32_t* nos, int64_t* xdoc_off,
                      const int64_t* len_dev = nullptr, const uint32_t* map = nullptr);
void launch_precompiled(hipStream_t st, const PcTables& pt, const uint8_t* text, int64_t n_bytes, const int64_t* doc_off, int64_t n_docs, const unsigned long long* verbatim,
                        const unsigned long long* bound, uint8_t* olen, uint16_t* ltot, uint32_t* wsum, uint32_t* bsum, uint32_t* wbase, int64_t* x_len, uint8_t* ntext,
                        uint32_t* nos, int64_t* ndoc_off, int* err, int grid, int64_t out_cap);
void launch_nfkc_normalize(hipStream_t st, const NfcTables& nt, const uint8_t* text, int64_t n_bytes, const int64_t* doc_off, int64_t n_docs, const unsigned long long* verbatim,
                           const unsigned long long* bound, uint8_t* olen, uint16_t* ltot, uint32_t* wsum, uint32_t* bsum, uint32_t* wbase, int64_t* x_len, uint8_t* ntext,
                           uint32_t* nos, int64_t* ndoc_off, int* err, int64_t out_cap);
void launch_pc_translate_matches(hipStream_t st, uint32_t* list, const uint32_t* n_list, const uint8_t* olen, const uint16_t* ltot, const uint32_t* wbase, int64_t n_bytes,
                                 const int64_t* x_len);
void launch_ms_units(hipStream_t st, const uint8_t* xtext, int64_t n_x, const int64_t* x_len, const unsigned long long* pmask, unsigned long long* startmask,
                     int64_t n_words, bool split);
void launch_ms_piece_rank(hipStream_t st, const unsigned long long* startmask, const uint32_t* wprefix, const unsigned long long* pmask, const uint32_t* pprefix,
                          int64_t n_x, const int64_t* x_len, uint32_t* pt_word);
void launch_translate_matches_norm(hipStream_t st, uint32_t* list, const uint32_t* n_list, const uint8_t* olen, const uint32_t* wbase, int64_t n_bytes, const int64_t* x_len);
void launch_translate_matches_prefix(hipStream_t st, uint32_t* list, const uint32_t* n_list, const unsigned long long* bmask, const uint32_t* wprefix, int64_t n_bytes,
                                     const int64_t* len_dev, const int64_t* total, const int64_t* xseg_off);
void launch_prefix_doc_csr(hipStream_t st, const int64_t* doc_off, int64_t n_docs, const unsigned long long* bmask, const uint32_t* wprefix, int64_t n_bytes,
                           const int64_t* len_dev, const int64_t* total, const int64_t* xseg_off, int64_t* xdoc_off);
void launch_mask_or(hipStream_t st, unsigned long long* dst, const unsigned long long* src, int64_t n_words, const uint32_t* n_list);
void launch_apply_matches(hipStream_t st, unsigned long long* startmask, unsigned long long* endmask, const unsigned long long* matchmask,
                          const unsigned long long* spanmask, const unsigned long long* stopmask, int64_t n_words, const uint32_t* n_list);
void launch_apply_match_ids(hipStream_t st, const uint32_t* match_list, const uint32_t* n_match, const unsigned long long* startmask,
                            const uint32_t* wprefix, uint32_t* tok0);
void launch_decode(hipStream_t st, const uint32_t* ids, const int64_t* tok_off, int64_t n_docs, int64_t n_tok, const void* entry, uint32_t n_ids,
                   const uint8_t* blob, uint32_t skip_special, uint32_t* firstmask, uint32_t* len, uint32_t* bsum, uint32_t* pos, int64_t* total,
                   int64_t* out_off, uint8_t* out_bytes_or_null, uint32_t from_end = 0, uint32_t* badmask = nullptr, uint32_t* dupmask = nullptr);
int prepare_long_kernel();
void launch_bpe_merge_long(hipStream_t st, int grid, const DevTables& t, const uint8_t* text, const QView& v, void* rows,
                           uint32_t* tmp_ids, uint32_t* tmp_end, uint32_t* list_huge, uint32_t* n_huge,
                           uint32_t* scratch, unsigned long long scratch_words, unsigned long long* scratch_used, int* err);
void launch_bpe_merge_long_only(hipStream_t st, int grid, const DevTables& t, const uint8_t* text, const QView& v, void* rows, uint32_t* tmp_ids, uint32_t* tmp_end,
                                uint32_t* list_huge, uint32_t* n_huge);
void launch_word_cache_insert(hipStream_t st, int grid, const DevTables& t, const uint8_t* text, const QView& v, const void* rows, const WordCache& wc);
void launch_compact(hipStream_t st, int grid, const uint32_t* tok0, const void* rows, const void* cache_rows, const uint32_t* tmp_ids, const int64_t* n_pretok,
                    unsigned long long* state, int64_t* n_tok, uint32_t* pt_tokoff, uint32_t* ids, const uint32_t* chunk_lo, const uint32_t* doc_pt,
                    int64_t n_docs, int64_t* tok_offsets, void* phases = nullptr, uint8_t* tok_b8 = nullptr);
int compact_grid(int n_cu);
void launch_zero_regions(hipStream_t st, int grid, const ZeroRegions& z);
void launch_zero_tail(hipStream_t st, uint8_t* p, const int64_t* len_dev, int n, unsigned long long* mask = nullptr, int64_t mask_words = 0, int grid = 1);
constexpr int CP_ITEMS_PER_LANE = 4;
constexpr int COMPACT_CHUNK = 256 * CP_ITEMS_PER_LANE;
constexpr int LB_GROUP_CHUNKS = 64, LB_GROUP_STRIDE = 32;
constexpr size_t lb_group_base(size_t n_chunks) { return (n_chunks + 15) & ~(size_t)15; }
constexpr size_t lb_state_words(size_t max_chunks) { return lb_group_base(max_chunks) + (max_chunks / LB_GROUP_CHUNKS + 1) * LB_GROUP_STRIDE; }
const char* test_hook(const char* name);

}
```

tokenizers_amd/csrc/kernels/bpe.hip:

```cpp


__device__ __forceinline__ void load_key16(const uint8_t* __restrict__ text, uint32_t s, uint32_t len, uint64_t* lo, uint64_t* hi) {
    const Unaligned16 v = *(const Unaligned16*)(text + s);
    uint32_t nl = min(len, 8u), nh = min(len, 16u) - nl;
    uint32_t m0 = nl >= 4 ? 0xFFFFFFFFu : ((1u << (8 * nl)) - 1u);
    uint32_t m1 = nl >= 8 ? 0xFFFFFFFFu : (nl > 4 ? ((1u << (8 * (nl - 4))) - 1u) : 0u);
    uint32_t m2 = nh >= 4 ? 0xFFFFFFFFu : ((1u << (8 * nh)) - 1u);
    uint32_t m3 = nh >= 8 ? 0xFFFFFFFFu : (nh > 4 ? ((1u << (8 * (nh - 4))) - 1u) : 0u);
    *lo = ((uint64_t)(v.b & m1) << 32) | (v.a & m0);
    *hi = ((uint64_t)(v.d & m3) << 32) | (v.c & m2);
}

constexpr uint32_t CLAIM_MAX_LEN = 32u;
constexpr uint32_t CLAIM_KEY_MAX = 15u;
__device__ __forceinline__ uint32_t claim_hash_long(uint32_t h16, uint32_t k4, uint32_t k5, uint32_t k6, uint32_t k7) {
    return mix32(h16 ^ (k4 * 0x9E3779B1u) ^ (k5 * 0x85EBCA77u) ^ (k6 * 0xC2B2AE3Du) ^ (k7 * 0x27D4EB2Fu));
}
__device__ __forceinline__ uint32_t claim_slot(uint32_t h, uint32_t mask) { return (word_hash2(h) >> 7) & mask; }
__device__ __forceinline__ uint32_t claim_slot_of(const uint8_t* __restrict__ text, uint32_t s, uint32_t len, uint32_t seed, uint32_t mask) {
    uint64_t lo, hi;
    load_key16(text, s, min(len, 16u), &lo, &hi);
    uint32_t h = word_hash1(lo, hi, len, seed);
    if (len > 16u) {
        uint64_t lo2, hi2;
// ... 126 lines not shown
        }
    }
}
template __global__ void k_bpe_merge<64>(DevTables, const uint8_t*, QView, uint4*, uint32_t*, uint32_t*);

__device__ __forceinline__ uint32_t select_bit32(uint32_t m, uint32_t k) {
    uint32_t pos = 0, c;
    c = __popc(m & 0xFFFFu); if (k >= c) { k -= c; pos += 16; m >>= 16; }
    c = __popc(m & 0xFFu);   if (k >= c) { k -= c; pos += 8;  m >>= 8; }
    c = __popc(m & 0xFu);    if (k >= c) { k -= c; pos += 4;  m >>= 4; }
    c = __popc(m & 0x3u);    if (k >= c) { k -= c; pos += 2;  m >>= 2; }
    c = m & 1u;              if (k >= c) { pos += 1; }
    return pos;
}

template <int S>
__global__ __launch_bounds__(256) void k_bpe_merge_lane(DevTables t, const uint8_t* __restrict__ text, QView v, uint4* __restrict__ rows,
                                                        uint32_t* __restrict__ tmp_ids, uint32_t* __restrict__ tmp_end) {
    __shared__ uint32_t s_qpre[NSQ + 1];
    constexpr uint32_t PB = (S == 16) ? 4 : 5;
    __shared__ uint32_t s_byte_id[256];
    __shared__ uint16_t s_disp[DISP_LDS_MAX];
    __shared__ uint32_t s_hist[S + 1];
    __shared__ uint4 s_sort[256];
    s_byte_id[threadIdx.x] = t.byte_id[threadIdx.x];
    const bool disp_in_lds = t.merge_bmask < (uint32_t)DISP_LDS_MAX;
    if (disp_in_lds)
        for (uint32_t i = threadIdx.x; i <= t.merge_bmask; i += 256) s_disp[i] = t.merge_disp[i];
    __syncthreads();
    const uint16_t* disp = disp_in_lds ? (const uint16_t*)s_disp : t.merge_disp;
    const uint32_t n_items = qview_prefix(v, s_qpre);
    const uint32_t stride = gridDim.x * 256;
    for (uint32_t base = blockIdx.x * 256; base < n_items; base += stride) {
        const uint32_t item = base + threadIdx.x;
        bool valid = item < n_items;
        uint32_t p = 0, s = 0, len = 0, claim = 0;
        if (valid) { p = qview_pos(s_qpre, v.sq_cap, item); const QItem it = v.q[p]; s = it.s; len = qitem_len(it.len); claim = it.len & QLEN_CLAIM; }
        valid = valid && len != 0u;
        {
            __syncthreads();
            if (threadIdx.x <= S) s_hist[threadIdx.x] = 0;
            __syncthreads();
            const uint32_t bin = valid ? len : (uint32_t)S;
            const uint32_t within = atomicAdd(&s_hist[bin], 1u);
            __syncthreads();
            uint32_t before = 0;
            for (uint32_t b = 0; b < bin; ++b) before += s_hist[b];
            const uint32_t slot = before + within;
            s_sort[slot] = make_uint4(p, s, len | claim, valid ? 1u : 0u);
            __syncthreads();
            const uint4 it = s_sort[threadIdx.x];
            p = it.x; s = it.y; len = qitem_len(it.z); claim = it.z & QLEN_CLAIM; valid = it.w != 0u;
        }
        uint64_t key[S / 8];
#pragma unroll
        for (int q = 0; q < S / 8; ++q) key[q] = 0;
        if (valid) {
            load_key16(text, s, min(len, 16u), &key[0], &key[1]);
            if (S == 32 && len > 16) load_key16(text, s + 16, len - 16, &key[S / 8 - 2], &key[S / 8 - 1]);
        }
        uint32_t ids[S], rk[S], nd[S];
#pragma unroll
        for (int i = 0; i < S; ++i) {
            uint32_t b = (uint32_t)((key[i / 8] >> (8 * (i % 8))) & 0xFFu);
            ids[i] = s_byte_id[b];
            rk[i] = RANK_NONE;
            nd[i] = 0;
        }
        if (t.byte_sfx) {
            const uint32_t sid = (valid && len) ? t.byte_sfx[text[s + len - 1u]] : 0u;
#pragma unroll
            for (int i = 0; i < S; ++i) ids[i] = (valid && (uint32_t)(i + 1) == len) ? sid : ids[i];
        }
#pragma unroll
        for (int i = 0; i < S - 1; ++i)
            if ((uint32_t)(i + 1) < len) merge_probe_d(t, disp, ids[i], ids[i + 1], &rk[i], &nd[i]);
        uint32_t n = len;
        uint32_t starts = (len >= 32) ? 0xFFFFFFFFu : ((1u << len) - 1u);
        bool active = valid && len > 1;
        while (__any(active)) {
            if (active) {
                uint32_t best = 0xFFFFFFFFu;
#pragma unroll
                for (int i = 0; i < S - 1; ++i) {
                    uint32_t k = (rk[i] << PB) | (uint32_t)i;
                    if ((uint32_t)(i + 1) < n && rk[i] != RANK_NONE) best = min(best, k);
                }
                if (best == 0xFFFFFFFFu) active = false;
                else {
                    const uint32_t w = best & (uint32_t)(S - 1);
                    uint32_t new_id = 0;
#pragma unroll
                    for (int i = 0; i < S - 1; ++i) new_id = ((uint32_t)i == w) ? nd[i] : new_id;
#pragma unroll
                    for (int i = 0; i < S; ++i) {
                        uint32_t nxt_id = (i + 1 < S) ? ids[i + 1] : 0u;
                        ids[i] = ((uint32_t)i == w) ? new_id : (((uint32_t)i > w) ? nxt_id : ids[i]);
                    }
#pragma unroll
                    for (int i = 0; i < S - 1; ++i) {
                        uint32_t nr = (i + 1 < S - 1) ? rk[i + 1] : RANK_NONE, nn = (i + 1 < S - 1) ? nd[i + 1] : 0u;
                        if ((uint32_t)i >= w) { rk[i] = nr; nd[i] = nn; }
                    }
                    if (tmp_end) starts &= ~(1u << select_bit32(starts, w + 1));
                    n -= 1;
                    uint32_t left = 0, right = 0;
#pragma unroll
                    for (int i = 0; i < S; ++i) {
                        left = ((uint32_t)i + 1 == w) ? ids[i] : left;
                        right = ((uint32_t)i == w + 1) ? ids[i] : right;
                    }
                    uint32_t r1 = RANK_NONE, n1 = 0, r2 = RANK_NONE, n2 = 0;
                    if (w > 0) merge_probe_d(t, disp, left, new_id, &r1, &n1);
                    if (w + 1 < n) merge_probe_d(t, disp, new_id, right, &r2, &n2);
#pragma unroll
                    for (int i = 0; i < S - 1; ++i) {
                        if ((uint32_t)i + 1 == w) { rk[i] = r1; nd[i] = n1; }
                        if ((uint32_t)i == w) { rk[i] = r2; nd[i] = n2; }
                    }
                    if (n < 2) active = false;
                }
            }
        }
        if (valid) {
            if (tmp_end && n >= 2u && n <= 4u) {
                uint32_t m = starts & (starts - 1u);
#pragma unroll
                for (int j = 1; j < 4; ++j)
                    if (m) { ids[j] |= row_boundary(text, s, (uint32_t)(__ffs(m) - 1), true); m &= m - 1u; }
            }
            { const uint4 row_ = make_row(n, s, ids[0], ids[1], ids[2], ids[3]); rows[v.row_base + p] = row_; TKAMD_PUBLISH_ROW(t, text, s, len | claim, row_); }
            if (n > 4u) {
#pragma unroll
                for (int j = 1; j < S; ++j)
                    if ((uint32_t)j < n) tmp_ids[s + j] = ids[j];
            }
            if (tmp_end) {
                uint32_t m = starts & (starts - 1u);
#pragma unroll
                for (int j = 0; j < S; ++j) {
                    if ((uint32_t)j < n) {
                        uint32_t e = m ? (uint32_t)(__ffs(m) - 1) : len;
                        tmp_end[s + j] = e;
                        m &= m - 1u;
                    }
                }
            }
        }
    }
}
template __global__ void k_bpe_merge_lane<16>(DevTables, const uint8_t*, QView, uint4*, uint32_t*, uint32_t*);
template __global__ void k_bpe_merge_lane<32>(DevTables, const uint8_t*, QView, uint4*, uint32_t*, uint32_t*);

template <int S, int NT, int NL, bool SYM_REGS, bool CHARS, bool TWO_Q>
__device__ __forceinline__ void bpe_merge_lds_unit(const DevTables& t, const uint8_t* __restrict__ text, const QView& v, const uint32_t* s_qpre, const uint32_t n_first,
                                                   const QView& v2, const uint32_t* s_qpre2, const uint32_t n_items, const uint32_t base, const uint32_t take,
                                                   uint32_t* lds_words, const uint16_t* const disp, uint32_t* s_probes, uint4* __restrict__ rows,
                                                   uint32_t* __restrict__ tmp_ids, uint32_t* __restrict__ tmp_end) {
    static_assert(NL <= NT && NL % 64 == 0 && 4 * NT <= S * NL, "whole wavefronts hold the words; the sort's items fit the key area");
    constexpr uint32_t PB = (S == 16) ? 4 : 5;
    uint32_t* const s_key = lds_words;
    uint32_t* const s_sym = s_key + S * NL;
    uint32_t* const s_byte_id = s_sym + (SYM_REGS ? 0 : S * NL);
    uint32_t* const s_hist = s_byte_id + 256;
    uint4* const s_sort = (uint4*)s_key;
    const uint32_t tid = threadIdx.x;
    const uint32_t item = base + tid;
    bool valid = tid < take && item < n_items;
    uint32_t s = 0, len = 0, qidx = 0, claim = 0;
    if (valid) {
        if (!TWO_Q || item < n_first) { const uint32_t qp = qview_pos(s_qpre, v.sq_cap, item); const QItem it = v.q[qp]; s = it.s; len = qitem_len(it.len); claim = it.len & QLEN_CLAIM; qidx = v.row_base + qp; }
        else { const uint32_t qp = qview_pos(s_qpre2, v2.sq_cap, item - n_first); const QItem it = v2.q[qp]; s = it.s; len = qitem_len(it.len); claim = it.len & QLEN_CLAIM; qidx = v2.row_base + qp; }
    }
    valid = valid && len != 0u;
    {
        __syncthreads();
        if (tid <= S + 1) s_hist[tid] = 0;
        __syncthreads();
        const uint32_t bin = valid ? len : (uint32_t)S + 1u;
        const uint32_t within = atomicAdd(&s_hist[bin], 1u);
        __syncthreads();
        uint32_t before = 0;
        for (uint32_t b = 0; b < bin; ++b) before += s_hist[b];
        s_sort[before + within] = make_uint4(claim, s, len, valid ? qidx + 1u : 0u);
        __syncthreads();
        const uint4 it = s_sort[tid];
        __syncthreads();
        claim = it.x; s = it.y; len = it.z; valid = it.w != 0u;
        qidx = it.w - 1u;
    }
    if (NL == NT || tid < NL) {
        uint32_t* my_key = s_key + tid;
        uint32_t* my_sym = s_sym + tid;
        uint32_t ids[S];
#define TKAMD_SYM_AT(dst, pos)                                                                 \
        do {                                                                                   \
            if (!SYM_REGS) (dst) = my_sym[(pos) * NL];                                         \
            else {                                                                             \
                (dst) = ids[0];                                                                \
                _Pragma("unroll") for (int q_ = 1; q_ < S; ++q_) (dst) = ((pos) == (uint32_t)q_) ? ids[q_] : (dst); \
            }                                                                                  \
        } while (0)
        uint32_t alive0 = 0u;
        {
            uint64_t kb[S / 8];
#pragma unroll
            for (int q = 0; q < S / 8; ++q) kb[q] = 0;
            if (valid) {
                load_key16(text, s, min(len, 16u), &kb[0], &kb[1]);
                if (S == 32 && len > 16) load_key16(text, s + 16, len - 16, &kb[S / 8 - 2], &kb[S / 8 - 1]);
            }
#define TKAMD_BYTE_AT(i_) ((i_) < S ? (uint32_t)((kb[((i_) < S ? (i_) : 0) / 8] >> (8 * (((i_) < S ? (i_) : 0) % 8))) & 0xFFu) : 0u)
            if (!CHARS) {
#pragma unroll
                for (int i = 0; i < S; ++i) {
                    ids[i] = s_byte_id[TKAMD_BYTE_AT(i)];
                    if (!SYM_REGS) my_sym[i * NL] = ids[i];
                }
                if (t.byte_sfx) {
                    const uint32_t sid = (valid && len) ? t.byte_sfx[text[s + len - 1u]] : 0u;
#pragma unroll
                    for (int i = 0; i < S; ++i) ids[i] = (valid && (uint32_t)(i + 1) == len) ? sid : ids[i];
                    if (!SYM_REGS && valid && len) my_sym[(len - 1u) * NL] = sid;
                }
                uint32_t wmax = valid ? len : 0u;
#pragma unroll
                for (int d_ = 32; d_ >= 1; d_ >>= 1) wmax = max(wmax, (uint32_t)__shfl_xor((int)wmax, d_, 64));
                wmax = (uint32_t)__builtin_amdgcn_readfirstlane((int)wmax);
                constexpr int PG = 8;
#pragma unroll
                for (int g = 0; g < S; g += PG) {
                    if ((uint32_t)(g + 1) < wmax) {
                        uint32_t rk[PG];
#pragma unroll
                        for (int q = 0; q < PG; ++q) {
                            const int i = g + q;
                            rk[q] = RANK_NONE;
                            if (i < S - 1) { uint32_t nd; merge_probe_d(t, disp, ids[i], ids[i + 1], &rk[q], &nd); }
                        }
#pragma unroll
                        for (int q = 0; q < PG; ++q) {
                            const int i = g + q;
                            my_key[i * NL] = ((uint32_t)(i + 1) < len && rk[q] != RANK_NONE) ? ((rk[q] << PB) | (uint32_t)i) : 0xFFFFFFFFu;
                        }
                    } else {
#pragma unroll
                        for (int q = 0; q < PG; ++q) my_key[(g + q) * NL] = 0xFFFFFFFFu;
                    }
                }
                alive0 = (len >= 32) ? 0xFFFFFFFFu : ((1u << len) - 1u);
            } else {
                static_assert(!CHARS || SYM_REGS, "the char start keeps its symbols in registers");
                uint32_t own[S];
#pragma unroll
                for (int i = 0; i < S; ++i) {
                    const uint32_t b0 = TKAMD_BYTE_AT(i), b1 = TKAMD_BYTE_AT(i + 1) & 0x3Fu, b2 = TKAMD_BYTE_AT(i + 2) & 0x3Fu, b3 = TKAMD_BYTE_AT(i + 3) & 0x3Fu;
                    const bool lead = (uint32_t)i < len && (b0 & 0xC0u) != 0x80u;
                    const uint32_t cl = b0 < 0x80u ? 1u : b0 < 0xE0u ? 2u : b0 < 0xF0u ? 3u : 4u;
                    const uint32_t cp = b0 < 0x80u ? b0 : b0 < 0xE0u ? ((b0 & 0x1Fu) << 6) | b1 : b0 < 0xF0u ? ((b0 & 0x0Fu) << 12) | (b1 << 6) | b2
                                                                                                              : ((b0 & 0x07u) << 18) | (b1 << 12) | (b2 << 6) | b3;
                    const uint32_t var = ((i != 0 && (t.cb & CB_PREFIX)) ? 1u : 0u) | (((uint32_t)i + cl >= len && (t.cb & CB_SUFFIX)) ? 2u : 0u);
                    own[i] = (lead && cp < 0x110000u) ? t.char_id[(cp << 2) | var] : CHAR_NONE;
                }
                bool unknown = false, prev_unk = false;
#pragma unroll
                for (int i = 0; i < S; ++i) {
                    ids[i] = 0u;
                    if ((uint32_t)i < len) {
                        const uint32_t b0 = TKAMD_BYTE_AT(i);
                        const bool lead = (b0 & 0xC0u) != 0x80u;
                        if (lead) unknown = own[i] == CHAR_NONE;
                        if (!unknown) { if (lead) { ids[i] = own[i]; alive0 |= 1u << i; prev_unk = false; } }
                        else if (t.cb & CB_BYTES) { ids[i] = s_byte_id[b0]; alive0 |= 1u << i; prev_unk = false; }
                        else if (lead) {
                            if (t.cb & CB_UNK) {
                                if (!(prev_unk && (t.cb & CB_FUSE))) { ids[i] = t.unk_id; alive0 |= 1u << i; }
                                prev_unk = true;
                            } else if (t.cb & CB_UNK_MISSING) atomicOr(t.err, ERR_UNK_OOV);
                        }
                    }
                }
#pragma unroll
                for (int i = 0; i < S; ++i) {
                    uint32_t k = 0xFFFFFFFFu;
                    const uint32_t above = (i < S - 1) ? (alive0 & ~((2u << i) - 1u)) : 0u;
                    if (((alive0 >> i) & 1u) && above) {
                        const uint32_t j = (uint32_t)__ffs(above) - 1u;
                        uint32_t right = ids[0];
#pragma unroll
                        for (int q_ = 1; q_ < S; ++q_) right = (j == (uint32_t)q_) ? ids[q_] : right;
                        uint32_t r, nd;
                        merge_probe_d(t, disp, ids[i], right, &r, &nd);
                        if (r != RANK_NONE) k = (r << PB) | (uint32_t)i;
                    }
                    my_key[i * NL] = k;
                }
            }
#undef TKAMD_BYTE_AT
        }
        uint32_t alive = alive0;
        bool active = valid && __popc(alive) > 1;
        while (__any(active)) {
            if (active) {
                uint32_t best = 0xFFFFFFFFu;
#pragma unroll
                for (int i = 0; i < S - 1; ++i) best = min(best, my_key[i * NL]);
                if (best == 0xFFFFFFFFu) active = false;
                else {
                    const uint32_t i = best & (uint32_t)(S - 1);
                    const uint32_t nid = (best >> PB) + t.newid_base;
                    uint32_t above = alive & ~((2u << i) - 1u);
                    const uint32_t j = (uint32_t)__ffs(above) - 1u;
                    above &= above - 1u;
                    alive &= ~(1u << j);
                    const uint32_t below = alive & ((1u << i) - 1u);
                    const bool has_k = above != 0u, has_h = below != 0u;
                    const uint32_t k = has_k ? (uint32_t)__ffs(above) - 1u : i;
                    const uint32_t h = has_h ? 31u - (uint32_t)__clz(below) : i;
                    uint32_t sr, sl;
                    TKAMD_SYM_AT(sr, k);
                    TKAMD_SYM_AT(sl, h);
                    if (SYM_REGS) {
#pragma unroll
                        for (int q = 0; q < S; ++q) ids[q] = (i == (uint32_t)q) ? nid : ids[q];
                    } else my_sym[i * NL] = nid;
                    uint32_t r1, r2;
                    merge_probe2_d(t, disp, sl, nid, nid, sr, &r1, &r2);
                    my_key[j * NL] = 0xFFFFFFFFu;
                    my_key[i * NL] = (has_k && r2 != RANK_NONE) ? ((r2 << PB) | i) : 0xFFFFFFFFu;
                    if (has_h) my_key[h * NL] = (r1 != RANK_NONE) ? ((r1 << PB) | h) : 0xFFFFFFFFu;
                    if (!has_k && !has_h) active = false;
                }
            }
        }
        if (valid) {
            const uint32_t c = (uint32_t)__popc(alive);
            uint32_t r[4] = {ids[0], 0u, 0u, 0u};
            if (!SYM_REGS) r[0] = my_sym[0];
            uint32_t m = alive & ~1u;
            if (CHARS) {
                m = alive;
                r[0] = 0u;
                if (m) { const uint32_t p0 = (uint32_t)__ffs(m) - 1u; TKAMD_SYM_AT(r[0], p0); m &= m - 1u; }
            }
            const bool carry = !CHARS && tmp_end != nullptr && c <= 4u;
#pragma unroll
            for (int j = 1; j < 4; ++j) {
                if (m) {
                    const uint32_t pos = (uint32_t)__ffs(m) - 1u;
                    TKAMD_SYM_AT(r[j], pos);
                    if (carry) r[j] |= row_boundary(text, s, pos, true);
                    else if (tmp_end) tmp_end[s + j - 1] = pos;
                    m &= m - 1u;
                }
            }
            if (m) {
                tmp_ids[s + 1] = r[1]; tmp_ids[s + 2] = r[2]; tmp_ids[s + 3] = r[3];
                for (uint32_t j = 4; m; m &= m - 1u, ++j) {
                    const uint32_t pos = (uint32_t)__ffs(m) - 1u;
                    uint32_t v_;
                    TKAMD_SYM_AT(v_, pos);
                    tmp_ids[s + j] = v_;
                    if (tmp_end) tmp_end[s + j - 1] = pos;
                }
            }
            if (tmp_end && c && !carry) tmp_end[s + c - 1] = len;
            { const uint4 row_ = make_row(c, s, r[0], r[1], r[2], r[3]); rows[qidx] = row_; TKAMD_PUBLISH_ROW(t, text, s, len | claim, row_); }
            if (t.probes) { const uint32_t k0 = (uint32_t)__popc(alive0); if (k0) atomicAdd(s_probes, (k0 - 1u) + 2u * (k0 - c)); }
        }
    }
}
#undef TKAMD_SYM_AT
template <int S, int NT, int NL, bool DISP_LDS, bool SYM_REGS>
__device__ __forceinline__ const uint16_t* bpe_merge_lds_tables(const DevTables& t, uint32_t* lds_words) {
    uint32_t* const s_byte_id = lds_words + (SYM_REGS ? 1 : 2) * S * NL;
    uint16_t* const s_disp = (uint16_t*)(s_byte_id + 256 + 64);
    const uint32_t tid = threadIdx.x;
    for (uint32_t i = tid; i < 256; i += NT) s_byte_id[i] = t.byte_id[i];
    if (DISP_LDS) {
        static_assert((DISP_LDS_MAX * 2) % 16 == 0, "whole 16-byte words");
        const uint32_t n16 = (t.merge_bmask + 8u) >> 3;
        for (uint32_t i = tid; i < n16; i += NT) ((uint4*)s_disp)[i] = ((const uint4*)t.merge_disp)[i];
    }
    __syncthreads();
    return DISP_LDS ? (const uint16_t*)s_disp : t.merge_disp;
}
template <int S, int NT, bool DISP_LDS, bool SYM_REGS, bool CHARS = false>
__global__ __launch_bounds__(NT) void k_bpe_merge_lds(DevTables t, const uint8_t* __restrict__ text, QView v, QView v2, uint4* __restrict__ rows,
                                                      uint32_t* __restrict__ tmp_ids, uint32_t* __restrict__ tmp_end) {
    __shared__ uint32_t s_qpre[NSQ + 1];
    __shared__ uint32_t s_qpre2[S == 32 ? NSQ + 1 : 1];
    __shared__ uint32_t s_probes;
    if (threadIdx.x == 0) s_probes = 0u;
    HIP_DYNAMIC_SHARED(__attribute__((aligned(16))) uint32_t, lds_words)
    const uint32_t n_first = qview_prefix(v, s_qpre);
    const uint16_t* const disp = bpe_merge_lds_tables<S, NT, NT, DISP_LDS, SYM_REGS>(t, lds_words);
    const uint32_t n_second = (S == 32 && v2.q) ? qview_prefix(v2, s_qpre2) : 0u;
    const uint32_t n_items = n_first + n_second;
    const uint32_t take = min((uint32_t)NT, ((n_items + gridDim.x - 1u) / gridDim.x + 63u) & ~63u);
    const uint32_t stride = gridDim.x * take;
    uint32_t round = 0u;
    for (uint32_t base0 = 0u; base0 < n_items; base0 += stride, ++round) {
        const uint32_t base = base0 + ((round & 1u) ? (gridDim.x - 1u - blockIdx.x) : blockIdx.x) * take;
        if (base >= n_items) { if (base0 + stride >= n_items) break; continue; }
        bpe_merge_lds_unit<S, NT, NT, SYM_REGS, CHARS, S == 32>(t, text, v, s_qpre, n_first, v2, s_qpre2, n_items, base, take, lds_words, disp, &s_probes, rows, tmp_ids, tmp_end);
    }
    if (t.probes) {
        __syncthreads();
        if (threadIdx.x == 0 && s_probes) atomicAdd(t.probes, s_probes);
    }
}
constexpr int PAIR_NT = 640, PAIR_NL32 = 320, PAIR_WG_PER_CU = 2;
static_assert(16 * PAIR_NT == 32 * PAIR_NL32, "one key area serves both roles");
template <bool DISP_LDS>
__global__ __launch_bounds__(PAIR_NT) void k_bpe_merge_lds_pair(DevTables t, const uint8_t* __restrict__ text, QView v16, QView v32, uint4* __restrict__ rows,
                                                                                      uint32_t* __restrict__ tmp_ids, uint32_t* __restrict__ tmp_end) {
    __shared__ uint32_t s_qpre16[NSQ + 1];
    __shared__ uint32_t s_qpre32[NSQ + 1];
    __shared__ uint32_t s_probes;
    if (threadIdx.x == 0) s_probes = 0u;
    HIP_DYNAMIC_SHARED(__attribute__((aligned(16))) uint32_t, lds_words)
    const uint32_t n16 = qview_prefix(v16, s_qpre16), n32 = qview_prefix(v32, s_qpre32);
    if (!(n16 | n32)) return;
    const uint16_t* const disp = bpe_merge_lds_tables<16, PAIR_NT, PAIR_NT, DISP_LDS, true>(t, lds_words);
    const uint32_t grid = gridDim.x;
    const uint32_t need_l = (n32 + PAIR_NL32 - 1u) / PAIR_NL32, need_s = (n16 + PAIR_NT - 1u) / PAIR_NT, need = need_l + need_s;
    const uint32_t rounds = (need + grid - 1u) / grid;
    const uint32_t slots = rounds * grid, spare = slots - need;
    const uint32_t slots_l = need_l + (spare * need_l + need - 1u) / need, slots_s = slots - slots_l;
    const bool spread = rounds == 1u;
    const uint32_t take_l = (n32 && spread) ? min((uint32_t)PAIR_NL32, ((n32 + slots_l - 1u) / slots_l + 63u) & ~63u) : (uint32_t)PAIR_NL32;
    const uint32_t take_s = (n16 && spread) ? min((uint32_t)PAIR_NT, ((n16 + slots_s - 1u) / slots_s + 63u) & ~63u) : (uint32_t)PAIR_NT;
    const uint32_t units_l = (n32 + take_l - 1u) / take_l, units = units_l + (n16 + take_s - 1u) / take_s;
    for (uint32_t round = 0u; round < rounds; ++round) {
        const uint32_t u = round * grid + ((round & 1u) ? (grid - 1u - blockIdx.x) : blockIdx.x);
        if (u < units_l)
            bpe_merge_lds_unit<32, PAIR_NT, PAIR_NL32, true, false, false>(t, text, v32, s_qpre32, n32, v32, s_qpre32, n32, u * take_l, take_l, lds_words, disp, &s_probes, rows, tmp_ids, tmp_end);
        else if (u < units)
            bpe_merge_lds_unit<16, PAIR_NT, PAIR_NT, true, false, false>(t, text, v16, s_qpre16, n16, v16, s_qpre16, n16, (u - units_l) * take_s, take_s, lds_words, disp, &s_probes, rows, tmp_ids, tmp_end);
    }
    if (t.probes) {
        __syncthreads();
        if (threadIdx.x == 0 && s_probes) atomicAdd(t.probes, s_probes);
    }
}
template __global__ void k_bpe_merge_lds_pair<true>(DevTables, const uint8_t*, QView, QView, uint4*, uint32_t*, uint32_t*);
template __global__ void k_bpe_merge_lds_pair<false>(DevTables, const uint8_t*, QView, QView, uint4*, uint32_t*, uint32_t*);
constexpr int lds_merge_bytes(int S, int NT, bool disp_lds, bool sym_regs) { return ((sym_regs ? 1 : 2) * S * NT + 256 + 64) * 4 + (disp_lds ? DISP_LDS_MAX * 2 : 0); }
template <int S, int NT, bool DISP_LDS, bool SYM_REGS>
static int prepare_lds_merge() {
    int rc = (int)hipFuncSetAttribute((const void*)k_bpe_merge_lds<S, NT, DISP_LDS, SYM_REGS, false>, hipFuncAttributeMaxDynamicSharedMemorySize, lds_merge_bytes(S, NT, DISP_LDS, SYM_REGS));
    if (rc == 0) rc = (int)hipFuncSetAttribute((const void*)k_bpe_merge_lds<S, NT, DISP_LDS, SYM_REGS, true>, hipFuncAttributeMaxDynamicSharedMemorySize, lds_merge_bytes(S, NT, DISP_LDS, SYM_REGS));
    return rc;
}
template <int S, int NT, bool DISP_LDS, bool SYM_REGS>
static void launch_lds_merge(hipStream_t st, int grid, const DevTables& t, const uint8_t* text, const QView& v, const QView& v2, uint4* rows, uint32_t* tmp_ids, uint32_t* tmp_end) {
    if (t.cb & CB_ON)
        hipLaunchKernelGGL((k_bpe_merge_lds<S, NT, DISP_LDS, SYM_REGS, true>), dim3(grid), dim3(NT), lds_merge_bytes(S, NT, DISP_LDS, SYM_REGS), st, t, text, v, v2, rows, tmp_ids, tmp_end);
    else
        hipLaunchKernelGGL((k_bpe_merge_lds<S, NT, DISP_LDS, SYM_REGS, false>), dim3(grid), dim3(NT), lds_merge_bytes(S, NT, DISP_LDS, SYM_REGS), st, t, text, v, v2, rows, tmp_ids, tmp_end);
}

static int pair_merge_wg_per_cu = PAIR_WG_PER_CU;
static int prepare_pair_merge() {
    const int lds = lds_merge_bytes(16, PAIR_NT, true, true);
    int rc = (int)hipFuncSetAttribute((const void*)k_bpe_merge_lds_pair<true>, hipFuncAttributeMaxDynamicSharedMemorySize, lds);
    if (rc == 0) rc = (int)hipFuncSetAttribute((const void*)k_bpe_merge_lds_pair<false>, hipFuncAttributeMaxDynamicSharedMemorySize, lds_merge_bytes(16, PAIR_NT, false, true));
    int n = 0, n_mem = 0;
    if (rc == 0) rc = (int)hipOccupancyMaxActiveBlocksPerMultiprocessor(&n, (const void*)k_bpe_merge_lds_pair<true>, PAIR_NT, (size_t)lds);
    if (rc == 0) rc = (int)hipOccupancyMaxActiveBlocksPerMultiprocessor(&n_mem, (const void*)k_bpe_merge_lds_pair<false>, PAIR_NT, (size_t)lds_merge_bytes(16, PAIR_NT, false, true));
    if (rc == 0 && (n < 1 || n_mem < 1)) rc = (int)hipErrorInvalidValue;
    if (rc == 0) pair_merge_wg_per_cu = std::min(std::min(n, n_mem), PAIR_WG_PER_CU);
    return rc;
}
int pair_merge_occupancy() { return pair_merge_wg_per_cu; }
static void launch_lds_merge_pair(hipStream_t st, int n_cu, const DevTables& t, const uint8_t* text, const QView& v16, const QView& v32, uint4* rows, uint32_t* tmp_ids, uint32_t* tmp_end) {
    const int grid = n_cu * pair_merge_wg_per_cu;
    if (t.merge_bmask < (uint32_t)DISP_LDS_MAX)
        hipLaunchKernelGGL(k_bpe_merge_lds_pair<true>, dim3(grid), dim3(PAIR_NT), lds_merge_bytes(16, PAIR_NT, true, true), st, t, text, v16, v32, rows, tmp_ids, tmp_end);
    else
        hipLaunchKernelGGL(k_bpe_merge_lds_pair<false>, dim3(grid), dim3(PAIR_NT), lds_merge_bytes(16, PAIR_NT, false, true), st, t, text, v16, v32, rows, tmp_ids, tmp_end);
}

__global__ __launch_bounds__(256) void k_bpe_merge_long(DevTables t, const uint8_t* __restrict__ text,
                                                        QView v, uint4* __restrict__ rows,
                                                        uint32_t* __restrict__ tmp_ids, uint32_t* __restrict__ tmp_end,
                                                        uint32_t* __restrict__ list_huge, uint32_t* __restrict__ n_huge) {
    __shared__ uint32_t s_qpre[NSQ + 1];
    HIP_DYNAMIC_SHARED(__attribute__((aligned(16))) uint8_t, lds_raw)
    uint32_t* sym = (uint32_t*)lds_raw;
    uint32_t* rnk = sym + LONG_PT_MAX;
    uint32_t* nid = rnk + LONG_PT_MAX;
    uint16_t* nxt = (uint16_t*)(nid + LONG_PT_MAX);
    uint16_t* prv = nxt + LONG_PT_MAX;
    __shared__ unsigned long long red[4];
    __shared__ uint32_t cnt_s;
    const int tid = (int)threadIdx.x;
    __shared__ uint32_t first_s;
    const uint32_t n = qview_prefix(v, s_qpre);
    for (uint32_t item = blockIdx.x; item < n; item += gridDim.x) {
        const uint32_t pos = qview_pos(s_qpre, v.sq_cap, item);
        const QItem it = v.q[pos];
        const uint32_t s = it.s, len = qitem_len(it.len);
        if (len == 0u) continue;
        if (len > (uint32_t)LONG_PT_MAX) {
            if (tid == 0) list_huge[atomicAdd(n_huge, 1u)] = pos;
            continue;
        }
        __syncthreads();
        if (!(t.cb & CB_ON)) {
            for (uint32_t i = tid; i < len; i += 256) {
                sym[i] = (t.byte_sfx && i + 1 == len) ? t.byte_sfx[text[s + i]] : t.byte_id[text[s + i]];
                nxt[i] = (i + 1 < len) ? (uint16_t)(i + 1) : (uint16_t)0xFFFF;
                prv[i] = (i > 0) ? (uint16_t)(i - 1) : (uint16_t)0xFFFF;
            }
        } else {
            for (uint32_t i = tid; i < len; i += 256) {
                const uint32_t b0 = text[s + i];
                uint32_t own = CHAR_NONE;
                if ((b0 & 0xC0u) != 0x80u) {
                    const uint32_t cl = b0 < 0x80u ? 1u : b0 < 0xE0u ? 2u : b0 < 0xF0u ? 3u : 4u;
                    uint32_t cp = b0 < 0x80u ? b0 : b0 < 0xE0u ? (b0 & 0x1Fu) : b0 < 0xF0u ? (b0 & 0x0Fu) : (b0 & 0x07u);
                    for (uint32_t q = 1; q < cl; ++q) cp = (cp << 6) | (i + q < len ? (text[s + i + q] & 0x3Fu) : 0u);
                    const uint32_t var = ((i != 0 && (t.cb & CB_PREFIX)) ? 1u : 0u) | ((i + cl >= len && (t.cb & CB_SUFFIX)) ? 2u : 0u);
                    if (cp < 0x110000u) own = t.char_id[(cp << 2) | var];
                }
                nid[i] = own;
                sym[i] = 0xFFFFFFFFu;
                nxt[i] = prv[i] = (uint16_t)0xFFFF;
                rnk[i] = RANK_NONE;
            }
            __syncthreads();
            if (tid == 0) {
                bool unknown = false, prev_unk = false;
                uint32_t last = 0xFFFFu;
                for (uint32_t i = 0; i < len; ++i) {
                    const uint32_t b0 = text[s + i];
                    const bool lead = (b0 & 0xC0u) != 0x80u;
                    if (lead) unknown = nid[i] == CHAR_NONE;
                    uint32_t id = 0xFFFFFFFFu;
                    if (!unknown) { if (lead) { id = nid[i]; prev_unk = false; } }
                    else if (t.cb & CB_BYTES) { id = t.byte_id[b0]; prev_unk = false; }
                    else if (lead) {
                        if (t.cb & CB_UNK) {
                            if (!(prev_unk && (t.cb & CB_FUSE))) id = t.unk_id;
                            prev_unk = true;
                        } else if (t.cb & CB_UNK_MISSING) atomicOr(t.err, ERR_UNK_OOV);
                    }
                    if (id != 0xFFFFFFFFu) {
                        sym[i] = id;
                        prv[i] = (uint16_t)last;
                        if (last != 0xFFFFu) nxt[last] = (uint16_t)i;
                        last = i;
                    }
                }
            }
        }
        __syncthreads();
        for (uint32_t i = tid; i < len; i += 256) {
            uint32_t r = RANK_NONE, ni = 0;
            const uint32_t j = nxt[i];
            if (sym[i] != 0xFFFFFFFFu && j != 0xFFFFu) merge_probe(t, sym[i], sym[j], &r, &ni);
            rnk[i] = r;
            nid[i] = ni;
        }
        __syncthreads();
        while (true) {
            unsigned long long best = ~0ull;
            for (uint32_t i = tid; i < len; i += 256) {
                uint32_t r = rnk[i];
                if (r != RANK_NONE) {
                    unsigned long long k = ((unsigned long long)r << 32) | i;
                    best = k < best ? k : best;
                }
            }
#pragma unroll
            for (int d = 32; d >= 1; d >>= 1) {
                unsigned long long o = __shfl_xor(best, d, 64);
                best = o < best ? o : best;
            }
            if ((tid & 63) == 0) red[tid >> 6] = best;
            __syncthreads();
            unsigned long long m01 = red[0] < red[1] ? red[0] : red[1];
            unsigned long long m23 = red[2] < red[3] ? red[2] : red[3];
            best = m01 < m23 ? m01 : m23;
            __syncthreads();
            if (best == ~0ull) break;
            if (tid == 0) {
                uint32_t w = (uint32_t)best;
                uint32_t r = nxt[w];
                uint32_t rn = nxt[r];
                sym[w] = nid[w];
                rnk[r] = RANK_NONE;
                sym[r] = 0xFFFFFFFFu;
                nxt[w] = (uint16_t)rn;
                if (rn != 0xFFFFu) prv[rn] = (uint16_t)w;
                uint32_t pw = prv[w];
                uint32_t r1 = RANK_NONE, n1 = 0, r2 = RANK_NONE, n2 = 0;
                if (pw != 0xFFFFu) merge_probe(t, sym[pw], sym[w], &r1, &n1);
                if (rn != 0xFFFFu) merge_probe(t, sym[w], sym[rn], &r2, &n2);
                if (pw != 0xFFFFu) { rnk[pw] = r1; nid[pw] = n1; }
                rnk[w] = r2;
                nid[w] = n2;
            }
            __syncthreads();
        }
        if (tid == 0) cnt_s = 0;
        __syncthreads();
        for (uint32_t base = 0; base < len; base += 256) {
            uint32_t i = base + tid;
            bool alive = i < len && sym[i] != 0xFFFFFFFFu;
            uint64_t bm = __ballot(alive);
            __shared__ uint32_t wcnt[4];
            if ((tid & 63) == 0) wcnt[tid >> 6] = (uint32_t)__popcll(bm);
            __syncthreads();
            uint32_t off = cnt_s;
            for (int w = 0; w < (tid >> 6); ++w) off += wcnt[w];
            if (alive) {
                uint32_t j = off + (uint32_t)mbcnt64(bm);
                if (j == 0) first_s = sym[i];
                else tmp_ids[s + j] = sym[i];
                if (tmp_end) {
                    uint32_t e = nxt[i];
                    tmp_end[s + j] = (e == 0xFFFFu) ? len : e;
                }
            }
            __syncthreads();
            if (tid == 0) cnt_s += wcnt[0] + wcnt[1] + wcnt[2] + wcnt[3];
            __syncthreads();
        }
        if (tid == 0) {
            const uint4 row_ = make_uint4((cnt_s ? first_s : 0u) | (ROW_CNT_MORE << ROW_CNT_SHIFT), s, cnt_s, 0u);
            rows[v.row_base + pos] = row_;
            TKAMD_PUBLISH_ROW(t, text, s, it.len, row_);
// ... 4 lines not shown
```

tokenizers_amd/csrc/kernels/launch.hip:

```cpp

void launch_mark_doc_starts_n(hipStream_t st, const int64_t* doc_off, int64_t n_docs, int64_t n_bytes, const int64_t* len_dev,
                              unsigned long long* docmask, int* err) {
    hipLaunchKernelGGL(k_mark_doc_starts, dim3(blocks_for(n_docs + 1, 256)), dim3(256), 0, st, doc_off, n_docs, n_bytes, len_dev, docmask, err);
}
void launch_mark_doc_starts(hipStream_t st, const int64_t* doc_off, int64_t n_docs, int64_t n_bytes,
                            unsigned long long* docmask, int* err) {
    launch_mark_doc_starts_n(st, doc_off, n_docs, n_bytes, nullptr, docmask, err);
}
void launch_validate_csr(hipStream_t st, const int64_t* doc_off, int64_t n_docs, int64_t n_bytes, int* err, int64_t* san) {
    hipLaunchKernelGGL(k_mark_doc_starts, dim3(blocks_for(n_docs + 1, 256)), dim3(256), 0, st, doc_off, n_docs, n_bytes, (const int64_t*)nullptr,
                       (unsigned long long*)nullptr, err);
    hipLaunchKernelGGL(k_sanitize_csr, dim3(blocks_for(n_docs + 1, 256)), dim3(256), 0, st, doc_off, n_docs, n_bytes, (const int*)err, san);
}
void launch_pretok_gpt2(hipStream_t st, const uint8_t* text, int64_t n_bytes, const int64_t* len_dev, const unsigned long long* docmask,
                        const uint16_t* uc1, const uint8_t* uc2, unsigned long long* startmask, unsigned long long* leadmask) {
    if (leadmask) hipLaunchKernelGGL((k_pretok_gpt2_seq<SQ_LUT_COPIES, true>), dim3(blocks_for((n_bytes >> 6) + 1, G2_WORDS_PER_BLOCK)), dim3(256), 0, st, text, n_bytes, len_dev, docmask, uc1, uc2, startmask, leadmask);
    else hipLaunchKernelGGL((k_pretok_gpt2_seq<SQ_LUT_COPIES, false>), dim3(blocks_for((n_bytes >> 6) + 1, G2_WORDS_PER_BLOCK)), dim3(256), 0, st, text, n_bytes, len_dev, docmask, uc1, uc2, startmask, (unsigned long long*)nullptr);
}
void launch_mask_scan(hipStream_t st, const unsigned long long* mask, int64_t n_words, uint32_t* bsum, uint32_t* wprefix,
                      int64_t* total, const int64_t* len_dev, uint32_t* tile_w) {
    unsigned nb = blocks_for(n_words, 256 * WS_PER);
    hipLaunchKernelGGL(k_words_reduce, dim3(nb), dim3(256), 0, st, mask, n_words, bsum, len_dev);
    hipLaunchKernelGGL(k_scan_single, dim3(1), dim3(1024), 0, st, bsum, (int64_t)nb, (const int64_t*)nullptr, (int64_t)1, total);
    hipLaunchKernelGGL(k_words_down, dim3(nb), dim3(256), 0, st, mask, n_words, (const uint32_t*)bsum, wprefix, len_dev, tile_w);
}
void launch_emit_pretok(hipStream_t st, const unsigned long long* startmask, const uint32_t* wprefix, int64_t n_bytes,
                        const int64_t* len_dev, const int64_t* n_pretok, uint32_t* pt_start) {
    hipLaunchKernelGGL(k_emit_pretok, dim3(blocks_for(n_bytes + 1, 4 * 4096)), dim3(256), 0, st, startmask, wprefix, n_bytes, len_dev, n_pretok, pt_start);
}
void launch_doc_first_pretok(hipStream_t st, const int64_t* doc_off, int64_t n_docs, int64_t n_bytes,
                             const unsigned long long* startmask, const uint32_t* wprefix, const int64_t* n_pretok, uint32_t* doc_pt, uint32_t* chunk_lo,
                             const int* err, int64_t* san) {
    hipLaunchKernelGGL(k_doc_first_pretok, dim3(blocks_for(n_docs + 1, 256)), dim3(256), 0, st, doc_off, n_docs, n_bytes, startmask, wprefix, n_pretok, doc_pt, chunk_lo,
                       (uint32_t)COMPACT_CHUNK, err, san);
}

void launch_lookup(hipStream_t st, int grid, const DevTables& t, const uint8_t* text, int64_t n_bytes, const int64_t* len_dev,
                   const unsigned long long* startmask, const unsigned long long* endmask, const uint32_t* wprefix, uint32_t* tok0,
                   const QueuePlan& plan, int* err, const unsigned long long* matchmask, const void* hot, const WordCache& wc,
                   uint32_t no_hits, uint32_t miss_is_unk, void* phases, uint32_t* counters) {
    LookupArgs a{};
    a.counters = counters;
    a.shortw = (const uint4*)t.shortw;
    a.shortw_mask = t.shortw_mask;
    a.shortw_bmask = t.shortw_bmask;
    a.shortw_disp = t.shortw_disp;
    a.shortw_k3 = t.shortw_k3;
    a.word_seed = t.word_seed;
    a.any_hit_final = t.ignore_merges;
    a.unk_id = t.unk_id;
    a.has_unk = t.has_unk;
    a.text = text;
    a.n_bytes_host = n_bytes;
    a.len_dev = len_dev;
    a.startmask = startmask;
    a.endmask = endmask;
    a.wprefix = wprefix;
    a.tok0 = tok0;
    for (int c = 0; c < 4; ++c) a.v[c] = plan.v[c];
    a.err = err;
    a.matchmask = matchmask;
    a.hot = (const uint4*)hot;
    a.cache_keys = wc.keys;
    a.claims = wc.claims;
    a.claim_mask = wc.claim_mask;
    a.no_hits = no_hits;
    a.miss_is_unk = miss_is_unk;
    a.phases = (unsigned long long*)phases;
    const int lds = lookup_lds_bytes();
    if (phases) { if (endmask) hipLaunchKernelGGL((k_lookup<true, true>), dim3(grid), dim3(LU_NT), lds, st, a); else hipLaunchKernelGGL((k_lookup<false, true>), dim3(grid), dim3(LU_NT), lds, st, a); }
    else if (endmask) hipLaunchKernelGGL((k_lookup<true, false>), dim3(grid), dim3(LU_NT), lds, st, a);
    else hipLaunchKernelGGL((k_lookup<false, false>), dim3(grid), dim3(LU_NT), lds, st, a);
}
void launch_bpe_merge(hipStream_t st, int grid, int group, const DevTables& t, const uint8_t* text, const QView& v, void* rows,
                      uint32_t* tmp_ids, uint32_t* tmp_end, const QView* also) {
    uint4* r = (uint4*)rows;
    const QView none{};
    const bool disp_fits = t.merge_bmask < (uint32_t)DISP_LDS_MAX;
    if (group == 5 && disp_fits) launch_lds_merge<16, 640, true, true>(st, grid * 2, t, text, v, none, r, tmp_ids, tmp_end);
    else if (group == 5) launch_lds_merge<16, 640, false, true>(st, grid * 2, t, text, v, none, r, tmp_ids, tmp_end);
    else if (group == 6 && disp_fits) launch_lds_merge<32, 768, true, true>(st, grid, t, text, v, also ? *also : none, r, tmp_ids, tmp_end);
    else if (group == 6) launch_lds_merge<32, 768, false, true>(st, grid, t, text, v, also ? *also : none, r, tmp_ids, tmp_end);
    else if (group == 1)
        hipLaunchKernelGGL(k_bpe_merge_lane<16>, dim3(grid), dim3(256), 0, st, t, text, v, r, tmp_ids, tmp_end);
    else if (group == 2)
        hipLaunchKernelGGL(k_bpe_merge_lane<32>, dim3(grid), dim3(256), 0, st, t, text, v, r, tmp_ids, tmp_end);
    else
        hipLaunchKernelGGL(k_bpe_merge<64>, dim3(grid), dim3(256), 0, st, t, text, v, r, tmp_ids, tmp_end);
}
void launch_bpe_merge_pair(hipStream_t st, int n_cu, const DevTables& t, const uint8_t* text, const QView& v16, const QView& v32, void* rows,
                           uint32_t* tmp_ids, uint32_t* tmp_end) {
    launch_lds_merge_pair(st, n_cu, t, text, v16, v32, (uint4*)rows, tmp_ids, tmp_end);
}
template <int KIND>
static void launch_pretok_local_t(hipStream_t st, const uint8_t* text, int64_t n_bytes, const int64_t* len_dev, const unsigned long long* docmask,
                                  const uint16_t* uc1, const uint8_t* uc2, unsigned long long* startmask, unsigned long long* endmask, bool len_bound) {
    hipLaunchKernelGGL(k_pretok_local_lane<KIND>, dim3(blocks_for(n_bytes + 2, 256 * PLW_MAIN)), dim3(256), 0, st, text, n_bytes, len_dev, docmask, uc1, uc2, startmask, endmask,
                       (len_bound && len_dev) ? 1 : 0);
}
void launch_pretok_local(hipStream_t st, int kind, const uint8_t* text, int64_t n_bytes, const int64_t* len_dev, const unsigned long long* docmask,
                         const uint16_t* uc1, const uint8_t* uc2, unsigned long long* startmask, unsigned long long* endmask, bool len_bound) {
    if (kind == PT_WHITESPACE) launch_pretok_local_t<PT_WHITESPACE>(st, text, n_bytes, len_dev, docmask, uc1, uc2, startmask, endmask, len_bound);
    else if (kind == PT_WHITESPACE_SPLIT) launch_pretok_local_t<PT_WHITESPACE_SPLIT>(st, text, n_bytes, len_dev, docmask, uc1, uc2, startmask, endmask, len_bound);
    else launch_pretok_local_t<PT_BERT>(st, text, n_bytes, len_dev, docmask, uc1, uc2, startmask, endmask, len_bound);
}
void launch_emit_pretok_end(hipStream_t st, const unsigned long long* startmask, const unsigned long long* endmask,
                            const uint32_t* wprefix, int64_t n_bytes, const int64_t* len_dev, uint32_t* pt_end) {
    hipLaunchKernelGGL(k_emit_pretok_end, dim3(blocks_for(n_bytes + 64, 4 * 4096)), dim3(256), 0, st, startmask, endmask, wprefix, n_bytes, len_dev, pt_end);
}
void launch_bert_normalize(hipStream_t st, const BnTables& bt, const uint8_t* text, int64_t n_bytes, const int64_t* doc_off, int64_t n_docs,
                           const unsigned long long* verbatim, uint8_t* olen, uint32_t* wsum, uint32_t* bsum, uint32_t* wbase, int64_t* x_len, uint8_t* ntext,
                           uint32_t* nos, uint32_t* noe, int64_t* ndoc_off, int* err) {
    const int64_t n_words = (n_bytes >> 6) + 1;
    uint8_t* const ltot = bn_ltot_of(olen, n_bytes);
    const BnOlen ol{olen, ltot};
    hipLaunchKernelGGL(k_bn_count, dim3(blocks_for(n_bytes + 1, 256 * BN_LANE)), dim3(256), 0, st, bt, text, n_bytes, verbatim, olen, ltot, wsum, err);

    unsigned nb = blocks_for(n_words, 256);
    hipLaunchKernelGGL(k_u32_reduce, dim3(nb), dim3(256), 0, st, (const uint32_t*)wsum, n_words, bsum);
    hipLaunchKernelGGL(k_scan_single, dim3(1), dim3(1024), 0, st, bsum, (int64_t)nb, (const int64_t*)nullptr, (int64_t)1, x_len);
    hipLaunchKernelGGL(k_u32_down, dim3(nb), dim3(256), 0, st, (const uint32_t*)wsum, n_words, (const uint32_t*)bsum, wbase);
    hipLaunchKernelGGL(k_bn_write, dim3(blocks_for(n_bytes, 256 * BN_LANE)), dim3(256), 0, st, bt, text, n_bytes, verbatim, ol, (const uint32_t*)wbase, ntext, nos, noe);
    if (!bt.chain)
        hipLaunchKernelGGL(k_bn_reorder_fix, dim3(std::min<unsigned>(blocks_for(n_bytes + 1, 256), 2048u)), dim3(256), 0, st, bt, text, n_bytes, verbatim, doc_off, n_docs,
                           ol, (const uint32_t*)wbase, ntext, nos, noe, err);
    hipLaunchKernelGGL(k_bn_doc_offsets, dim3(blocks_for(n_docs + 1, 256)), dim3(256), 0, st, doc_off, n_docs, n_bytes, ol,
                       (const uint32_t*)wbase, (const int64_t*)x_len, ndoc_off);
}
void launch_nfc_check(hipStream_t st, const NfcTables& nt, const uint8_t* text, int64_t n_bytes, int* note) {
    hipLaunchKernelGGL(k_nfc_check, dim3(blocks_for(n_bytes, 256 * NFC_LANE)), dim3(256), 0, st, nt, text, n_bytes, note);
}
void launch_nfc_bound(hipStream_t st, unsigned long long* dmask, const unsigned long long* verbatim, int64_t n_words) {
    hipLaunchKernelGGL(k_nfc_bound, dim3(blocks_for(n_words, 256)), dim3(256), 0, st, dmask, verbatim, n_words);
}
void launch_nfc_normalize(hipStream_t st, const NfcTables& nt, const uint8_t* text, int64_t n_bytes, const int64_t* doc_off, int64_t n_docs,
                          const unsigned long long* verbatim, const unsigned long long* bound, uint8_t* olen, uint32_t* wsum, uint32_t* bsum, uint32_t* wbase,
                          int64_t* x_len, uint8_t* ntext, uint32_t* nos, int64_t* ndoc_off, int* err) {
    const int64_t n_words = (n_bytes >> 6) + 1;
    uint8_t* const ltot = bn_ltot_of(olen, n_bytes);
    const BnOlen ol{olen, ltot};
    const NfcArgs a{nt, text, n_bytes, verbatim, bound};
    hipLaunchKernelGGL(k_nfc_count, dim3(blocks_for(n_bytes + 1, 256 * NFC_LANE)), dim3(256), 0, st, a, olen, ltot, wsum, err);
    unsigned nb = blocks_for(n_words, 256);
    hipLaunchKernelGGL(k_u32_reduce, dim3(nb), dim3(256), 0, st, (const uint32_t*)wsum, n_words, bsum);
    hipLaunchKernelGGL(k_scan_single, dim3(1), dim3(1024), 0, st, bsum, (int64_t)nb, (const int64_t*)nullptr, (int64_t)1, x_len);
    hipLaunchKernelGGL(k_u32_down, dim3(nb), dim3(256), 0, st, (const uint32_t*)wsum, n_words, (const uint32_t*)bsum, wbase);
    hipLaunchKernelGGL(k_nfc_write, dim3(blocks_for(n_bytes, 256 * NFC_LANE)), dim3(256), 0, st, a, ol, (const uint32_t*)wbase, (const int*)err, ntext, nos);
    hipLaunchKernelGGL(k_bn_doc_offsets, dim3(blocks_for(n_docs + 1, 256)), dim3(256), 0, st, doc_off, n_docs, n_bytes, ol,
                       (const uint32_t*)wbase, (const int64_t*)x_len, ndoc_off);
}
void launch_metaspace(hipStream_t st, const uint8_t* text, int64_t n_bytes, const int64_t* doc_off, int64_t n_docs, const unsigned long long* pstart,
                      const unsigned long long* dstart, const unsigned long long* mmask, const unsigned long long* smask, uint32_t prepend, uint8_t* olen,
                      uint32_t* wsum, uint32_t* bsum, uint32_t* wbase, int64_t* x_len, uint8_t* xtext, uint32_t* nos, int64_t* xdoc_off, const int64_t* len_dev,
                      const uint32_t* map) {
    const int64_t n_words = (n_bytes >> 6) + 1;
    uint8_t* const ltot = bn_ltot_of(olen, n_bytes);
    const BnOlen ol{olen, ltot};
    const MsArgs a{text, n_bytes, pstart, dstart, mmask, smask, prepend, len_dev, map};
    hipLaunchKernelGGL(k_ms_count, dim3(blocks_for(n_bytes + 1, 256 * BN_LANE)), dim3(256), 0, st, a, olen, ltot, wsum);
    unsigned nb = blocks_for(n_words, 256);
    hipLaunchKernelGGL(k_u32_reduce, dim3(nb), dim3(256), 0, st, (const uint32_t*)wsum, n_words, bsum);
    hipLaunchKernelGGL(k_scan_single, dim3(1), dim3(1024), 0, st, bsum, (int64_t)nb, (const int64_t*)nullptr, (int64_t)1, x_len);
    hipLaunchKernelGGL(k_u32_down, dim3(nb), dim3(256), 0, st, (const uint32_t*)wsum, n_words, (const uint32_t*)bsum, wbase);
    hipLaunchKernelGGL(k_ms_write, dim3(blocks_for(n_bytes, 256 * BN_LANE)), dim3(256), 0, st, a, ol, (const uint32_t*)wbase, xtext, nos);
    hipLaunchKernelGGL(k_bn_doc_offsets, dim3(blocks_for(n_docs + 1, 256)), dim3(256), 0, st, doc_off, n_docs, n_bytes, ol,
                       (const uint32_t*)wbase, (const int64_t*)x_len, xdoc_off);
}
void launch_precompiled(hipStream_t st, const PcTables& pt, const uint8_t* text, int64_t n_bytes, const int64_t* doc_off, int64_t n_docs, const unsigned long long* verbatim,
                        const unsigned long long* bound, uint8_t* olen, uint16_t* ltot, uint32_t* wsum, uint32_t* bsum, uint32_t* wbase, int64_t* x_len, uint8_t* ntext,
                        uint32_t* nos, int64_t* ndoc_off, int* err, int grid, int64_t out_cap) {
    const int64_t n_words = (n_bytes >> 6) + 1;
    const PcOlen ol{olen, ltot};
    const PcArgs a{pt, text, n_bytes, verbatim, bound};
    hipLaunchKernelGGL(k_pc_count, dim3(blocks_for(n_bytes + 1, 256 * PC_LANE)), dim3(256), 0, st, a, olen, ltot, wsum, err);
    unsigned nb = blocks_for(n_words, 256);
    hipLaunchKernelGGL(k_u32_reduce, dim3(nb), dim3(256), 0, st, (const uint32_t*)wsum, n_words, bsum);
    hipLaunchKernelGGL(k_scan_single, dim3(1), dim3(1024), 0, st, bsum, (int64_t)nb, (const int64_t*)nullptr, (int64_t)1, x_len);
    hipLaunchKernelGGL(k_u32_down, dim3(nb), dim3(256), 0, st, (const uint32_t*)wsum, n_words, (const uint32_t*)bsum, wbase);
    hipLaunchKernelGGL(k_pc_check_len, dim3(1), dim3(64), 0, st, x_len, out_cap, err);
    hipLaunchKernelGGL(k_pc_write, dim3(blocks_for(n_bytes, 256 * PC_LANE)), dim3(256), 0, st, a, ol, (const uint32_t*)wbase, (const int64_t*)x_len, ntext, nos);
    if (nos) hipLaunchKernelGGL(k_pc_lost_fix, dim3(std::min<unsigned>(blocks_for(n_words, 256), (unsigned)std::max(1, grid))), dim3(256), 0, st, a, ol, (const uint32_t*)wbase,
                                (const int64_t*)x_len, (const int*)err, nos);
    hipLaunchKernelGGL(k_pc_doc_offsets, dim3(blocks_for(n_docs + 1, 256)), dim3(256), 0, st, doc_off, n_docs, n_bytes, ol, (const uint32_t*)wbase, (const int64_t*)x_len, ndoc_off);
}
void launch_pc_translate_matches(hipStream_t st, uint32_t* list, const uint32_t* n_list, const uint8_t* olen, const uint16_t* ltot, const uint32_t* wbase, int64_t n_bytes,
                                 const int64_t* x_len) {
    hipLaunchKernelGGL(k_pc_translate_matches, dim3(256), dim3(256), 0, st, list, n_list, PcOlen{olen, ltot}, wbase, n_bytes, x_len);
}
void launch_nfkc_normalize(hipStream_t st, const NfcTables& nt, const uint8_t* text, int64_t n_bytes, const int64_t* doc_off, int64_t n_docs, const unsigned long long* verbatim,
                           const unsigned long long* bound, uint8_t* olen, uint16_t* ltot, uint32_t* wsum, uint32_t* bsum, uint32_t* wbase, int64_t* x_len, uint8_t* ntext,
                           uint32_t* nos, int64_t* ndoc_off, int* err, int64_t out_cap) {
    const int64_t n_words = (n_bytes >> 6) + 1;
    const PcOlen ol{olen, ltot};
    const NfcArgs a{nt, text, n_bytes, verbatim, bound};
    hipLaunchKernelGGL(k_nfkc_count, dim3(blocks_for(n_bytes + 1, 256 * NFC_LANE)), dim3(256), 0, st, a, olen, ltot, wsum, err);
    unsigned nb = blocks_for(n_words, 256);
    hipLaunchKernelGGL(k_u32_reduce, dim3(nb), dim3(256), 0, st, (const uint32_t*)wsum, n_words, bsum);
    hipLaunchKernelGGL(k_scan_single, dim3(1), dim3(1024), 0, st, bsum, (int64_t)nb, (const int64_t*)nullptr, (int64_t)1, x_len);
    hipLaunchKernelGGL(k_u32_down, dim3(nb), dim3(256), 0, st, (const uint32_t*)wsum, n_words, (const uint32_t*)bsum, wbase);
    hipLaunchKernelGGL(k_pc_check_len, dim3(1), dim3(64), 0, st, x_len, out_cap, err);
    hipLaunchKernelGGL(k_nfkc_write, dim3(blocks_for(n_bytes, 256 * NFC_LANE)), dim3(256), 0, st, a, ol, (const uint32_t*)wbase, (const int64_t*)x_len, (const int*)err, ntext, nos);
    hipLaunchKernelGGL(k_pc_doc_offsets, dim3(blocks_for(n_docs + 1, 256)), dim3(256), 0, st, doc_off, n_docs, n_bytes, ol, (const uint32_t*)wbase, (const int64_t*)x_len, ndoc_off);
}
void launch_ms_units(hipStream_t st, const uint8_t* xtext, int64_t n_x, const int64_t* x_len, const unsigned long long* pmask, unsigned long long* startmask,
                     int64_t n_words, bool split) {
    hipLaunchKernelGGL(k_ms_units, dim3(blocks_for(n_words, 256)), dim3(256), 0, st, xtext, n_x, x_len, pmask, startmask, n_words, split ? 1u : 0u);
}
void launch_ms_piece_rank(hipStream_t st, const unsigned long long* startmask, const uint32_t* wprefix, const unsigned long long* pmask, const uint32_t* pprefix,
                          int64_t n_x, const int64_t* x_len, uint32_t* pt_word) {
    hipLaunchKernelGGL(k_ms_piece_rank, dim3(blocks_for((n_x >> 6) + 1, 256)), dim3(256), 0, st, startmask, wprefix, pmask, pprefix, n_x, x_len, pt_word);
}
void launch_long_vocab3(hipStream_t st, int grid, const DevTables& t, const uint8_t* text, const QView& v1, const QView& v2, const QView& v3, void* rows, uint32_t miss_is_unk,
                        int* err, const WordCache& wc) {
    hipLaunchKernelGGL(k_long_vocab3, dim3(3 * grid), dim3(256), 0, st, t, text, v1, v2, v3, (uint4*)rows, miss_is_unk, err, wc.claim_mask,
                       wc.claims ? (uint4*)wc.rows : (uint4*)nullptr, wc.claim_pos);
}
void launch_wordpiece_all(hipStream_t st, int grid_short, int grid_long, const DevTables& t, const uint8_t* text, const QueuePlan& plan, void* rows, uint32_t* tmp_ids,
                          uint32_t* tmp_end, int* err) {
    hipLaunchKernelGGL(k_wordpiece_all, dim3(3 * grid_long + grid_short), dim3(256), 0, st, t, text, plan.v[0], plan.v[1], plan.v[2], plan.v[3], (uint4*)rows, tmp_ids, tmp_end, err,
                       (uint32_t)(3 * grid_long));
}
void launch_unigram_all(hipStream_t st, int grid_short, int grid_long, const DevTables& t, const uint8_t* text, const QueuePlan& plan, void* rows, uint32_t* tmp_ids,
                        uint32_t* tmp_end, int* err, void* state) {
    hipLaunchKernelGGL(k_unigram_all, dim3(3 * grid_long + grid_short), dim3(256), 0, st, t, text, plan.v[0], plan.v[1], plan.v[2], plan.v[3], (uint4*)rows, tmp_ids, tmp_end, err,
                       (uint4*)state, (uint32_t)(3 * grid_long));
}
void launch_unigram_run_offsets(hipStream_t st, int grid, const DevTables& t, const uint32_t* ids, uint32_t* offsets, const int64_t* tok_offsets, int64_t n_docs,
                                const int64_t* n_tok, uint8_t* flags) {
    hipLaunchKernelGGL(k_unigram_run_flags, dim3(grid), dim3(256), 0, st, ids, (const uint32_t*)offsets, n_tok, t.uni_is_byte, t.uni_n_ids, flags);
    hipLaunchKernelGGL(k_unigram_run_offsets, dim3(grid), dim3(256), 0, st, offsets, tok_offsets, n_docs, n_tok, (const uint8_t*)flags);
}
void launch_pretok_llama3(hipStream_t st, const uint8_t* text, int64_t n_bytes, const int64_t* len_dev, const unsigned long long* docmask,
                          const uint16_t* uc1, const uint8_t* uc2, unsigned long long* startmask, unsigned long long* slowmask,
                          const int64_t* doc_off, int64_t n_docs, const int64_t* n_docs_dev, uint32_t* slow_docs, uint32_t* n_slow_docs,
                          SplitRule rule, const uint16_t* ucc1, const uint8_t* ucc2, unsigned long long* tileflags, unsigned long long* leadmask) {
    const L3Seq q{uc1, uc2, ucc1, ucc2, rule};
    const unsigned doc_blocks = std::min<unsigned>(blocks_for(n_docs, 256), 4096u);
    if (split_rule_fast(rule)) {
        if (leadmask) hipLaunchKernelGGL((k_pretok_llama3_lane<false, true>), dim3(blocks_for(n_bytes + 1, 256 * L3W_MAIN)), dim3(256), 0, st, text, n_bytes, len_dev, docmask, uc1, uc2, startmask, slowmask, rule,
                           (const uint16_t*)nullptr, (const uint8_t*)nullptr, tileflags, leadmask);
        else hipLaunchKernelGGL((k_pretok_llama3_lane<false, false>), dim3(blocks_for(n_bytes + 1, 256 * L3W_MAIN)), dim3(256), 0, st, text, n_bytes, len_dev, docmask, uc1, uc2, startmask, slowmask, rule,
                           (const uint16_t*)nullptr, (const uint8_t*)nullptr, tileflags, (unsigned long long*)nullptr);
        const unsigned n_tiles = blocks_for(n_bytes + 1, PT_TILE);
        hipLaunchKernelGGL(k_pretok_llama3, dim3(tileflags ? blocks_for(n_tiles, 64) : n_tiles), dim3(256), 0, st, text, n_bytes, len_dev, docmask, uc1, uc2, startmask, slowmask,
                           (const unsigned long long*)tileflags, rule);
// ... 187 lines not shown
```

tokenizers_amd/tokenizer.py:

```python
from __future__ import annotations

import ctypes as C
import json
import os
import re
import threading
from typing import Iterable, Sequence

import numpy as np

from . import _lib
from ._lib import DeviceError, TokenizersAmdError, UnsupportedError


try:
    from . import _marshal
except ImportError:
    _marshal = None


_FORKED = [False]
os.register_at_fork(after_in_child=lambda: _FORKED.__setitem__(0, True))


# ... 790 lines not shown
        offs = wids = None
        if offsets != "none":
            offs = view(self._lib.tkamd_batch_offsets(b), C.c_uint32, (nt, 2), np.uint32)
        if word_ids:
            wids = view(self._lib.tkamd_batch_word_ids(b), C.c_uint32, (nt,), np.uint32)
        pads = None
        pp = self._lib.tkamd_batch_pad_counts(b)
        if pp:
            pads = view(pp, C.c_uint32, (n_docs,), np.uint32)
        be = BatchEncoding(ids, to, offs, wids, self._id_to_token(), self._specials if add_special_tokens else (0, 0), pads,
                           self.info["padding"] == 2, self.info["pad_type_id"], self._pad_token)
        be._no_seq_ranges = self._no_post_processor
        be.kinds = kinds
        tp = self._lib.tkamd_batch_type_ids(b)
        if tp or pairs:
            be.type_ids = view(tp, C.c_uint8, (nt,), np.uint8)
            if pairs:
                be.seq_ids = view(self._lib.tkamd_batch_sequence_ids(b), C.c_uint8, (nt,), np.uint8)
        ed = self._lib.tkamd_batch_encoding_docs(b)
        if ed:
            be.enc_docs = view(ed, C.c_uint32, (n_docs,), np.uint32)
            be._first = np.searchsorted(be.enc_docs, np.arange(n_inputs, dtype=np.uint32), side="left")
            ep = self._lib.tkamd_batch_encoding_parts(b)
            if ep:
                be.enc_parts = view(ep, C.c_uint32, (n_docs, 2), np.uint32)
        return be

    def encode_file(self, path: str, offsets: str = "none", word_ids: bool = False, add_special_tokens: bool = False) -> BatchEncoding:
        buf, off = read_lines(path)
        return self.encode_packed(buf, off, offsets, word_ids, add_special_tokens)

    def encode(self, sequence, pair=None, is_pretokenized: bool = False, add_special_tokens: bool = True) -> Encoding:
        item = sequence if pair is None else (sequence, pair)
        return self.encode_batch([item], is_pretokenized=is_pretokenized, add_special_tokens=add_special_tokens)[0]

    def _encode_any(self, input, offsets: str, word_ids: bool, add_special_tokens: bool, is_pretokenized: bool):
        inputs = input if isinstance(input, (list, tuple)) else list(input)
        if is_pretokenized:
            is_pair = lambda it: isinstance(it, (tuple, list)) and len(it) == 2 and all(isinstance(x, (list, tuple)) for x in it)
        else:
            is_pair = lambda it: isinstance(it, (tuple, list))
        overflowing = self.info["truncation"] >= 0
        first = is_pair(inputs[0]) if len(inputs) else False
        if len(inputs) < 2 or len(inputs) > 4096 or all(is_pair(it) == first for it in inputs):
            try:
                return self.encode_batch_csr(inputs, offsets=offsets, word_ids=word_ids, add_special_tokens=add_special_tokens,
                                             is_pretokenized=is_pretokenized, overflowing=overflowing)
            except (UnsupportedError, TypeError):
                if len(inputs) <= 4096 or all(is_pair(it) == first for it in inputs):
                    raise
        return self._encode_mixed(inputs, offsets, word_ids, add_special_tokens, is_pretokenized, overflowing, is_pair)

    def _encode_mixed(self, inputs, offsets, word_ids, add_special_tokens, is_pretokenized, overflowing, is_pair) -> BatchEncoding:
        seqs: list = []
        inp_off = [0]
        kinds = np.zeros(len(inputs), dtype=np.uint8)
        for i, it in enumerate(inputs):
            if is_pair(it):
                if len(it) != 2:
                    raise UnsupportedError("an input is a sequence or a pair of sequences")
                seqs.extend(it)
                kinds[i] = 1
            else:
                seqs.append(it)
            inp_off.append(len(seqs))
        seq_off = None
        if is_pretokenized:
            words: list[str] = []
            seq_off = [0]
            for sq in seqs:
                if not (isinstance(sq, (list, tuple)) and all(isinstance(x, str) for x in sq)):
                    raise TypeError("is_pretokenized=True: every sequence must be a list of str (TextInputSequence / PreTokenizedInputSequence)")
                words.extend(sq)
                seq_off.append(len(words))
            seqs = words
        elif not all(isinstance(x, str) for x in seqs):
            raise UnsupportedError("a batch holds single sequences (str) and pairs (str, str); lists of words need is_pretokenized=True")
        flags = self._flags(offsets, word_ids, add_special_tokens, False, overflowing)
        inp = np.asarray(inp_off, dtype=np.int64)
        b = C.c_void_p()
        with self._stage_lock:
            buf, doc_off = self._pack_staged(seqs)
            so = np.asarray(seq_off, dtype=np.int64) if seq_off is not None else None
            _lib.check(self._lib.tkamd_encode_batch_mixed(self._h, buf.ctypes.data, doc_off.ctypes.data, len(doc_off) - 1,
                                                          so.ctypes.data if so is not None else None, len(so) - 1 if so is not None else -1,
                                                          inp.ctypes.data, len(inputs), flags, C.byref(b)))
        return self._wrap_batch(b, len(inputs), offsets, word_ids, add_special_tokens, True, kinds)

    def encode_batch(self, input: Iterable[str], is_pretokenized: bool = False, add_special_tokens: bool = True) -> BatchEncoding:
        return self._encode_any(input, "char", True, add_special_tokens, is_pretokenized)

    def encode_batch_fast(self, input: Iterable[str], is_pretokenized: bool = False, add_special_tokens: bool = True) -> BatchEncoding:
        return self._encode_any(input, "none", False, add_special_tokens, is_pretokenized)

    def decode_batch_csr(self, ids: np.ndarray, tok_offsets: np.ndarray, skip_special_tokens: bool = True) -> tuple[np.ndarray, np.ndarray]:
        ids = np.ascontiguousarray(ids, dtype=np.uint32)
        tok_offsets = np.ascontiguousarray(tok_offsets, dtype=np.int64)
        n_docs = len(tok_offsets) - 1
        if n_docs < 0:
            raise ValueError("tok_offsets must hold n_docs + 1 entries")
        b = C.c_void_p()
        flags = _lib.SKIP_SPECIAL if skip_special_tokens else 0
        _lib.check(self._lib.tkamd_decode_batch(self._h, ids.ctypes.data, tok_offsets.ctypes.data, n_docs, flags, C.byref(b)))
        try:
            nb = self._lib.tkamd_text_n_bytes(b)
            raw = np.ctypeslib.as_array(C.cast(self._lib.tkamd_text_bytes(b), C.POINTER(C.c_uint8)), shape=(max(nb, 1),))[:nb].copy()
            off = np.ctypeslib.as_array(C.cast(self._lib.tkamd_text_doc_offsets(b), C.POINTER(C.c_int64)), shape=(n_docs + 1,)).copy()
        finally:
            self._lib.tkamd_text_free(b)
        return raw, off

    def decode_token(self, token_id: int, first_position: bool = False) -> tuple[bytes, int]:
        ln, fl = C.c_int32(0), C.c_int32(0)
        buf = (C.c_uint8 * 4096)()
        _lib.check(self._lib.tkamd_decode_token(self._h, int(token_id), int(first_position), buf, 4096, C.byref(ln), C.byref(fl)))
        return bytes(buf[:min(ln.value, 4096)]), fl.value

    def decode_batch(self, sequences: Sequence[Sequence[int]], skip_special_tokens: bool = True) -> list[str]:
        ids, off = pack_id_sequences(sequences)
        raw, doff = self.decode_batch_csr(ids, off, skip_special_tokens)
        buf = raw.tobytes()
        return [buf[doff[i]:doff[i + 1]].decode("utf-8", "replace") for i in range(len(sequences))]

    def decode(self, ids: Sequence[int], skip_special_tokens: bool = True) -> str:
        return self.decode_batch([ids], skip_special_tokens)[0]

    def encode_batch_device(self, d_text_ptr: int, d_doc_offsets_ptr: int, n_docs: int, n_bytes: int,
                            offsets: str = "none", word_ids: bool = False, stream: int = 0, unsynced: bool = False) -> DeviceBatch:
        flags = {"none": _lib.OFFSETS_NONE, "byte": _lib.OFFSETS_BYTE, "char": _lib.OFFSETS_CHAR}[offsets]
        if word_ids:
            flags |= _lib.WANT_WORD_IDS
        if unsynced:
            flags |= _lib.NO_SPECULATION
        res = _lib.DeviceResult()
        _lib.check(self._lib.tkamd_encode_batch_device(self._h, d_text_ptr, d_doc_offsets_ptr, n_docs, n_bytes, flags,
                                                       stream, C.byref(res)))
        return DeviceBatch(self, res, n_docs, stream, capacity=int(res.ids_capacity))

    def word_cache(self, enable: bool = True, clear: bool = False) -> None:
        _lib.check(self._lib.tkamd_word_cache(self._h, 1 if enable else 0, 1 if clear else 0))
        self._word_cache_on = bool(enable)

    def shard_stats(self) -> list[tuple[int, int, float]]:
        n = max(len(self.devices), 1)
        nb, ms, k = (C.c_int64 * n)(), (C.c_double * n)(), C.c_int(0)
        _lib.check(self._lib.tkamd_shard_stats(self._h, nb, ms, n, C.byref(k)))
        return [(self.devices[i], nb[i], ms[i]) for i in range(min(k.value, n))]

    def profile(self, on: bool) -> None:
        _lib.check(self._lib.tkamd_profile_enable(self._h, 1 if on else 0))
        self._profile_on = bool(on)

    def queue_sizes(self) -> dict[str, int]:
        arr = (C.c_uint32 * 22)()
        _lib.check(self._lib.tkamd_profile_counters(self._h, arr, 22))
        out = {"merge16": arr[0], "merge32": arr[3], "merge64": arr[1], "merge_long": arr[2], "pretok_slow_docs": arr[4], "merge_huge": arr[7]}
        if arr[5]:
            out["claim_candidates"], out["claim_shared"] = arr[5], arr[6]
        out["added_spec_pause"] = arr[14]
        out["nfc_spec_pause"], out["nfc_reruns"] = arr[16], arr[17]
        out["merge_pair_wg_per_cu"] = arr[13]
        out["q16_div"] = arr[15]
        out["shortw_slots"], out["shortw_buckets"], out["shortw_max_disp"], out["merge_slots"] = arr[18], arr[19], arr[20], arr[21]
        if arr[12]:
            out["merge_probes"] = arr[12]
        return out

    def debug_phases(self, reset: bool = True) -> dict[str, list[int]]:
        out = {}
        for which, name in ((0, "lookup"), (1, "compact")):
            arr = (C.c_uint64 * 8)()
            _lib.check(self._lib.tkamd_debug_phases(self._h, which, arr, 1 if reset else 0))
            out[name] = list(arr)
        return out

    def profile_read(self, reset: bool = True) -> dict[str, tuple[float, int]]:
        arr = (_lib.StageTime * _lib.MAX_STAGES)()
        n = C.c_int(0)
        _lib.check(self._lib.tkamd_profile_read(self._h, arr, _lib.MAX_STAGES, C.byref(n), 1 if reset else 0))
        return {arr[i].name.decode(): (arr[i].ms_total, arr[i].launches) for i in range(n.value)}
```

Measured before the change: 282.6.

## Rework pair merge kernel: binary-tree register select, batched probes, new work plan

Measured after the change: 288.3 (median of 6 runs). 1.02x the previous value.

```diff
diff --git a/tokenizers_amd/csrc/capi/api_handle.cpp b/tokenizers_amd/csrc/capi/api_handle.cpp
--- a/tokenizers_amd/csrc/capi/api_handle.cpp
+++ b/tokenizers_amd/csrc/capi/api_handle.cpp
@@ -31,6 +31,7 @@
         if (const char* e = test_hook("TKAMD_NFC_SPEC")) t->nfc_spec_len = std::max(0, atoi(e));
         t->cp_grid = compact_grid(t->n_cu);
         if (const char* e = test_hook("TKAMD_CP_GRID")) t->cp_grid = std::max(1, atoi(e));
+        if (const char* e = test_hook("TKAMD_MERGE_PAIR_GRID")) t->pair_grid = std::max(1, atoi(e));
         t->devices.push_back(device);
     }
     return t;
diff --git a/tokenizers_amd/csrc/capi/handle.cpp b/tokenizers_amd/csrc/capi/handle.cpp
--- a/tokenizers_amd/csrc/capi/handle.cpp
+++ b/tokenizers_amd/csrc/capi/handle.cpp
@@ -49,6 +49,7 @@
     int64_t last_n_enc = -1;
     int last_ntok_slot = 1;
     uint32_t last_counters[CNT_COUNT] = {0};
+    uint32_t last_pair_grid = 0;
     bool force_general = false;
     bool force_nfc = false;
     bool last_note_nfc = false;
@@ -86,6 +87,7 @@
     int n_direct = 0;
     int n_hot = 0;
     uint32_t shortw_max_disp = 0;
+    int pair_grid = 0;
     int cp_grid = 0;
     std::atomic<int> claims_pause{0};
     std::atomic<int> added_spec_pause{0};
diff --git a/tokenizers_amd/csrc/capi/pipeline.cpp b/tokenizers_amd/csrc/capi/pipeline.cpp
--- a/tokenizers_amd/csrc/capi/pipeline.cpp
+++ b/tokenizers_amd/csrc/capi/pipeline.cpp
@@ -772,6 +772,7 @@
         const char* const pair_hook = test_hook("TKAMD_MERGE_PAIR");
         const bool pair = can_one && !(pair_hook && pair_hook[0] == '0');
         const bool one = can_one && !pair;
+        w->last_pair_grid = 0u;
         const size_t huge_words = std::min<size_t>((size_t)6 * N + 4096, (size_t)1 << 28);
         const bool huge_possible = N > (size_t)LONG_PT_MAX;
         if (huge_possible) {
@@ -805,7 +806,7 @@
         } else {
             if (pair) {
                 pf.begin("bpe_merge_lds_pair");
-                launch_bpe_merge_pair(st, t->n_cu, mdt, x_text, plan.v[0], plan.v[1], w->w_rows.p, w->w_tmp_ids.as<uint32_t>(), tmp_end);
+                w->last_pair_grid = (uint32_t)launch_bpe_merge_pair(st, t->n_cu, t->pair_grid, mdt, x_text, plan.v[0], plan.v[1], w->w_rows.p, w->w_tmp_ids.as<uint32_t>(), tmp_end);
                 pf.end();
             } else {
                 pf.begin(lds ? "bpe_merge_lds32" : "bpe_merge_lane32");
diff --git a/tokenizers_amd/csrc/capi/probes.cpp b/tokenizers_amd/csrc/capi/probes.cpp
--- a/tokenizers_amd/csrc/capi/probes.cpp
+++ b/tokenizers_amd/csrc/capi/probes.cpp
@@ -245,6 +245,7 @@
         if (!w) return TKAMD_OK;
         for (int i = 0; i < n && i < CNT_COUNT; ++i) out[i] = w->last_counters[i];
         if (n > 13) out[13] = (uint32_t)pair_merge_occupancy();
+        if (n > 22) out[22] = w->last_pair_grid;
         if (n > 14) out[14] = (uint32_t)std::max(0, t->added_spec_pause.load());
         if (n > 15) out[15] = t->q16_div;
         if (n > 16) out[16] = (uint32_t)std::max(0, t->nfc_spec_pause.load());
diff --git a/tokenizers_amd/csrc/kernels.hip b/tokenizers_amd/csrc/kernels.hip
--- a/tokenizers_amd/csrc/kernels.hip
+++ b/tokenizers_amd/csrc/kernels.hip
@@ -8,6 +8,7 @@
 #include "device_utils.hpp"
 #include "kernels.hpp"
 #include "overflow_core.hpp"
+#include "merge_pair_plan_core.hpp"
 #include "bert_norm_core.hpp"
 #include "nfc_core.hpp"
 #include "precompiled_core.hpp"
diff --git a/tokenizers_amd/csrc/kernels.hpp b/tokenizers_amd/csrc/kernels.hpp
--- a/tokenizers_amd/csrc/kernels.hpp
+++ b/tokenizers_amd/csrc/kernels.hpp
@@ -299,7 +299,7 @@
                    uint32_t no_hits, uint32_t miss_is_unk, void* phases = nullptr, uint32_t* counters = nullptr);
 void launch_bpe_merge(hipStream_t st, int grid, int group, const DevTables& t, const uint8_t* text, const QView& v, void* rows,
                       uint32_t* tmp_ids, uint32_t* tmp_end, const QView* also = nullptr);
-void launch_bpe_merge_pair(hipStream_t st, int n_cu, const DevTables& t, const uint8_t* text, const QView& v16, const QView& v32, void* rows,
+int launch_bpe_merge_pair(hipStream_t st, int n_cu, int grid_hook, const DevTables& t, const uint8_t* text, const QView& v16, const QView& v32, void* rows,
                            uint32_t* tmp_ids, uint32_t* tmp_end);
 int pair_merge_occupancy();
 inline size_t bn_olen_bytes(int64_t n_bytes) { return (((size_t)n_bytes + 64 + 15) & ~(size_t)15) + ((size_t)n_bytes >> 4) + 64; }
diff --git a/tokenizers_amd/csrc/kernels/bpe.hip b/tokenizers_amd/csrc/kernels/bpe.hip
--- a/tokenizers_amd/csrc/kernels/bpe.hip
+++ b/tokenizers_amd/csrc/kernels/bpe.hip
@@ -302,6 +302,8 @@
 template __global__ void k_bpe_merge_lane<16>(DevTables, const uint8_t*, QView, uint4*, uint32_t*, uint32_t*);
 template __global__ void k_bpe_merge_lane<32>(DevTables, const uint8_t*, QView, uint4*, uint32_t*, uint32_t*);
 
+__device__ __forceinline__ uint32_t sel32(bool c, uint32_t a, uint32_t b) { return c ? a : b; }
+
 template <int S, int NT, int NL, bool SYM_REGS, bool CHARS, bool TWO_Q>
 __device__ __forceinline__ void bpe_merge_lds_unit(const DevTables& t, const uint8_t* __restrict__ text, const QView& v, const uint32_t* s_qpre, const uint32_t n_first,
                                                    const QView& v2, const uint32_t* s_qpre2, const uint32_t n_items, const uint32_t base, const uint32_t take,
@@ -347,10 +349,16 @@
         do {                                                                                   \
             if (!SYM_REGS) (dst) = my_sym[(pos) * NL];                                         \
             else {                                                                             \
-                (dst) = ids[0];                                                                \
-                _Pragma("unroll") for (int q_ = 1; q_ < S; ++q_) (dst) = ((pos) == (uint32_t)q_) ? ids[q_] : (dst); \
+                const bool b0_ = ((pos) & 1u) != 0u, b1_ = ((pos) & 2u) != 0u, b2_ = ((pos) & 4u) != 0u, b3_ = ((pos) & 8u) != 0u; \
+                const uint32_t lo_ = TKAMD_SEL16(0);                                           \
+                (dst) = (S == 32) ? sel32(((pos) & 16u) != 0u, TKAMD_SEL16(16), lo_) : lo_;    \
             }                                                                                  \
         } while (0)
+#define TKAMD_SEL1(i_) ids[(i_) < S ? (i_) : 0]
+#define TKAMD_SEL2(i_) sel32(b0_, TKAMD_SEL1((i_) + 1), TKAMD_SEL1(i_))
+#define TKAMD_SEL4(i_) sel32(b1_, TKAMD_SEL2((i_) + 2), TKAMD_SEL2(i_))
+#define TKAMD_SEL8(i_) sel32(b2_, TKAMD_SEL4((i_) + 4), TKAMD_SEL4(i_))
+#define TKAMD_SEL16(i_) sel32(b3_, TKAMD_SEL8((i_) + 8), TKAMD_SEL8(i_))
         uint32_t alive0 = 0u;
         {
             uint64_t kb[S / 8];
@@ -381,12 +389,26 @@
 #pragma unroll
                 for (int g = 0; g < S; g += PG) {
                     if ((uint32_t)(g + 1) < wmax) {
-                        uint32_t rk[PG];
+                        uint32_t rk[PG], slot[PG];
+                        uint4 x[PG];
+#pragma unroll
+                        for (int q = 0; q < PG; ++q) {
+                            const int i = g + q;
+                            slot[q] = 0u;
+                            if (i < S - 1) slot[q] = ph_slot(merge_hash2(ids[i], ids[i + 1], t.merge_seed), disp[merge_hash1(ids[i], ids[i + 1], t.merge_seed) & t.merge_bmask], t.merge_mask);
+                        }
+                        __builtin_amdgcn_sched_barrier(0);
+#pragma unroll
+                        for (int q = 0; q < PG; ++q) {
+                            x[q] = make_uint4(0u, 0u, 0u, 0u);
+                            if (g + q < S - 1) x[q] = ((const uint4*)t.merges)[slot[q]];
+                        }
+                        __builtin_amdgcn_sched_barrier(0);
 #pragma unroll
                         for (int q = 0; q < PG; ++q) {
                             const int i = g + q;
                             rk[q] = RANK_NONE;
-                            if (i < S - 1) { uint32_t nd; merge_probe_d(t, disp, ids[i], ids[i + 1], &rk[q], &nd); }
+                            if (i < S - 1) rk[q] = (x[q].x == ids[i] && x[q].y == ids[i + 1]) ? x[q].z : RANK_NONE;
                         }
 #pragma unroll
                         for (int q = 0; q < PG; ++q) {
@@ -450,7 +472,8 @@
         }
         uint32_t alive = alive0;
         bool active = valid && __popc(alive) > 1;
-        while (__any(active)) {
+        do {
+            uint32_t at = (uint32_t)S, at_id = 0u;
             if (active) {
                 uint32_t best = 0xFFFFFFFFu;
 #pragma unroll
@@ -470,10 +493,8 @@
                     uint32_t sr, sl;
                     TKAMD_SYM_AT(sr, k);
                     TKAMD_SYM_AT(sl, h);
-                    if (SYM_REGS) {
-#pragma unroll
-                        for (int q = 0; q < S; ++q) ids[q] = (i == (uint32_t)q) ? nid : ids[q];
-                    } else my_sym[i * NL] = nid;
+                    if (SYM_REGS) { at = i; at_id = nid; }
+                    else my_sym[i * NL] = nid;
                     uint32_t r1, r2;
                     merge_probe2_d(t, disp, sl, nid, nid, sr, &r1, &r2);
                     my_key[j * NL] = 0xFFFFFFFFu;
@@ -482,7 +503,11 @@
                     if (!has_k && !has_h) active = false;
                 }
             }
-        }
+            if (SYM_REGS) {
+#pragma unroll
+                for (int q = 0; q < S; ++q) ids[q] = sel32(at == (uint32_t)q, at_id, ids[q]);
+            }
+        } while (__any(active));
         if (valid) {
             const uint32_t c = (uint32_t)__popc(alive);
             uint32_t r[4] = {ids[0], 0u, 0u, 0u};
@@ -521,6 +546,11 @@
     }
 }
 #undef TKAMD_SYM_AT
+#undef TKAMD_SEL16
+#undef TKAMD_SEL8
+#undef TKAMD_SEL4
+#undef TKAMD_SEL2
+#undef TKAMD_SEL1
 template <int S, int NT, int NL, bool DISP_LDS, bool SYM_REGS>
 __device__ __forceinline__ const uint16_t* bpe_merge_lds_tables(const DevTables& t, uint32_t* lds_words) {
     uint32_t* const s_byte_id = lds_words + (SYM_REGS ? 1 : 2) * S * NL;
@@ -562,6 +592,7 @@
 }
 constexpr int PAIR_NT = 640, PAIR_NL32 = 320, PAIR_WG_PER_CU = 2;
 static_assert(16 * PAIR_NT == 32 * PAIR_NL32, "one key area serves both roles");
+static_assert(PAIR_NT == (int)PAIR_TAKE_S_MAX && PAIR_NL32 == (int)PAIR_TAKE_L_MAX, "the plan's units are the kernel's");
 template <bool DISP_LDS>
 __global__ __launch_bounds__(PAIR_NT) void k_bpe_merge_lds_pair(DevTables t, const uint8_t* __restrict__ text, QView v16, QView v32, uint4* __restrict__ rows,
                                                                                       uint32_t* __restrict__ tmp_ids, uint32_t* __restrict__ tmp_end) {
@@ -574,20 +605,13 @@
     if (!(n16 | n32)) return;
     const uint16_t* const disp = bpe_merge_lds_tables<16, PAIR_NT, PAIR_NT, DISP_LDS, true>(t, lds_words);
     const uint32_t grid = gridDim.x;
-    const uint32_t need_l = (n32 + PAIR_NL32 - 1u) / PAIR_NL32, need_s = (n16 + PAIR_NT - 1u) / PAIR_NT, need = need_l + need_s;
-    const uint32_t rounds = (need + grid - 1u) / grid;
-    const uint32_t slots = rounds * grid, spare = slots - need;
-    const uint32_t slots_l = need_l + (spare * need_l + need - 1u) / need, slots_s = slots - slots_l;
-    const bool spread = rounds == 1u;
-    const uint32_t take_l = (n32 && spread) ? min((uint32_t)PAIR_NL32, ((n32 + slots_l - 1u) / slots_l + 63u) & ~63u) : (uint32_t)PAIR_NL32;
-    const uint32_t take_s = (n16 && spread) ? min((uint32_t)PAIR_NT, ((n16 + slots_s - 1u) / slots_s + 63u) & ~63u) : (uint32_t)PAIR_NT;
-    const uint32_t units_l = (n32 + take_l - 1u) / take_l, units = units_l + (n16 + take_s - 1u) / take_s;
-    for (uint32_t round = 0u; round < rounds; ++round) {
-        const uint32_t u = round * grid + ((round & 1u) ? (grid - 1u - blockIdx.x) : blockIdx.x);
-        if (u < units_l)
-            bpe_merge_lds_unit<32, PAIR_NT, PAIR_NL32, true, false, false>(t, text, v32, s_qpre32, n32, v32, s_qpre32, n32, u * take_l, take_l, lds_words, disp, &s_probes, rows, tmp_ids, tmp_end);
-        else if (u < units)
-            bpe_merge_lds_unit<16, PAIR_NT, PAIR_NT, true, false, false>(t, text, v16, s_qpre16, n16, v16, s_qpre16, n16, (u - units_l) * take_s, take_s, lds_words, disp, &s_probes, rows, tmp_ids, tmp_end);
+    const PairPlan plan = pair_plan(n16, n32, grid);
+    for (uint32_t round = 0u; round < plan.rounds; ++round) {
+        const uint32_t u = pair_plan_unit(round, blockIdx.x, grid);
+        if (u < plan.units_l)
+            bpe_merge_lds_unit<32, PAIR_NT, PAIR_NL32, true, false, false>(t, text, v32, s_qpre32, n32, v32, s_qpre32, n32, u * plan.take_l, plan.take_l, lds_words, disp, &s_probes, rows, tmp_ids, tmp_end);
+        else if (u < plan.units)
+            bpe_merge_lds_unit<16, PAIR_NT, PAIR_NT, true, false, false>(t, text, v16, s_qpre16, n16, v16, s_qpre16, n16, (u - plan.units_l) * plan.take_s, plan.take_s, lds_words, disp, &s_probes, rows, tmp_ids, tmp_end);
     }
     if (t.probes) {
         __syncthreads();
@@ -624,12 +648,13 @@
     return rc;
 }
 int pair_merge_occupancy() { return pair_merge_wg_per_cu; }
-static void launch_lds_merge_pair(hipStream_t st, int n_cu, const DevTables& t, const uint8_t* text, const QView& v16, const QView& v32, uint4* rows, uint32_t* tmp_ids, uint32_t* tmp_end) {
-    const int grid = n_cu * pair_merge_wg_per_cu;
+static int launch_lds_merge_pair(hipStream_t st, int n_cu, int grid_hook, const DevTables& t, const uint8_t* text, const QView& v16, const QView& v32, uint4* rows, uint32_t* tmp_ids, uint32_t* tmp_end) {
+    const int grid = grid_hook > 0 ? grid_hook : n_cu * pair_merge_wg_per_cu;
     if (t.merge_bmask < (uint32_t)DISP_LDS_MAX)
         hipLaunchKernelGGL(k_bpe_merge_lds_pair<true>, dim3(grid), dim3(PAIR_NT), lds_merge_bytes(16, PAIR_NT, true, true), st, t, text, v16, v32, rows, tmp_ids, tmp_end);
     else
         hipLaunchKernelGGL(k_bpe_merge_lds_pair<false>, dim3(grid), dim3(PAIR_NT), lds_merge_bytes(16, PAIR_NT, false, true), st, t, text, v16, v32, rows, tmp_ids, tmp_end);
+    return grid;
 }
 
 __global__ __launch_bounds__(256) void k_bpe_merge_long(DevTables t, const uint8_t* __restrict__ text,
diff --git a/tokenizers_amd/csrc/kernels/launch.hip b/tokenizers_amd/csrc/kernels/launch.hip
--- a/tokenizers_amd/csrc/kernels/launch.hip
+++ b/tokenizers_amd/csrc/kernels/launch.hip
@@ -88,9 +88,9 @@
     else
         hipLaunchKernelGGL(k_bpe_merge<64>, dim3(grid), dim3(256), 0, st, t, text, v, r, tmp_ids, tmp_end);
 }
-void launch_bpe_merge_pair(hipStream_t st, int n_cu, const DevTables& t, const uint8_t* text, const QView& v16, const QView& v32, void* rows,
+int launch_bpe_merge_pair(hipStream_t st, int n_cu, int grid_hook, const DevTables& t, const uint8_t* text, const QView& v16, const QView& v32, void* rows,
                            uint32_t* tmp_ids, uint32_t* tmp_end) {
-    launch_lds_merge_pair(st, n_cu, t, text, v16, v32, (uint4*)rows, tmp_ids, tmp_end);
+    return launch_lds_merge_pair(st, n_cu, grid_hook, t, text, v16, v32, (uint4*)rows, tmp_ids, tmp_end);
 }
 template <int KIND>
 static void launch_pretok_local_t(hipStream_t st, const uint8_t* text, int64_t n_bytes, const int64_t* len_dev, const unsigned long long* docmask,
diff --git a/tokenizers_amd/csrc/merge_pair_plan_core.hpp b/tokenizers_amd/csrc/merge_pair_plan_core.hpp
--- /dev/null
+++ b/tokenizers_amd/csrc/merge_pair_plan_core.hpp
@@ -0,0 +1,51 @@
+#pragma once
+#include <cstdint>
+
+#include "tables.hpp"
+
+namespace tkamd {
+
+constexpr uint32_t PAIR_TAKE_S_MAX = 640u;
+constexpr uint32_t PAIR_TAKE_L_MAX = 320u;
+constexpr uint32_t PAIR_TAKE_L_THIN = 256u;
+
+struct PairPlan {
+    uint32_t rounds;
+    uint32_t take_l;
+    uint32_t take_s;
+    uint32_t units_l;
+    uint32_t units;
+};
+
+TK_HD uint32_t pair_plan_up64(uint32_t x) { return (x + 63u) & ~63u; }
+
+TK_HD PairPlan pair_plan(uint32_t n16, uint32_t n32, uint32_t grid) {
+    PairPlan p;
+    const uint32_t need_l = (n32 + PAIR_TAKE_L_MAX - 1u) / PAIR_TAKE_L_MAX, need_s = (n16 + PAIR_TAKE_S_MAX - 1u) / PAIR_TAKE_S_MAX;
+    const uint32_t need = need_l + need_s;
+    p.rounds = (need + grid - 1u) / grid;
+    p.take_l = PAIR_TAKE_L_MAX;
+    p.take_s = PAIR_TAKE_S_MAX;
+    if (p.rounds == 1u) {
+        if (n32) {
+            const uint32_t slots_l = grid - need_s;
+            const uint32_t thin = pair_plan_up64((n32 + slots_l - 1u) / slots_l);
+            p.take_l = thin <= PAIR_TAKE_L_THIN ? thin : PAIR_TAKE_L_MAX;
+        }
+        const uint32_t units_l = (n32 + p.take_l - 1u) / p.take_l;
+        if (n16) {
+            const uint32_t slots_s = grid - units_l;
+            const uint32_t even = pair_plan_up64((n16 + slots_s - 1u) / slots_s);
+            p.take_s = even < PAIR_TAKE_S_MAX ? even : PAIR_TAKE_S_MAX;
+        }
+    }
+    p.units_l = (n32 + p.take_l - 1u) / p.take_l;
+    p.units = p.units_l + (n16 + p.take_s - 1u) / p.take_s;
+    return p;
+}
+
+TK_HD uint32_t pair_plan_unit(uint32_t round, uint32_t wg, uint32_t grid) {
+    return round * grid + ((round & 1u) ? (grid - 1u - wg) : wg);
+}
+
+}
diff --git a/tokenizers_amd/tokenizer.py b/tokenizers_amd/tokenizer.py
--- a/tokenizers_amd/tokenizer.py
+++ b/tokenizers_amd/tokenizer.py
@@ -966,14 +966,15 @@
         self._profile_on = bool(on)
 
     def queue_sizes(self) -> dict[str, int]:
-        arr = (C.c_uint32 * 22)()
-        _lib.check(self._lib.tkamd_profile_counters(self._h, arr, 22))
+        arr = (C.c_uint32 * 23)()
+        _lib.check(self._lib.tkamd_profile_counters(self._h, arr, 23))
         out = {"merge16": arr[0], "merge32": arr[3], "merge64": arr[1], "merge_long": arr[2], "pretok_slow_docs": arr[4], "merge_huge": arr[7]}
         if arr[5]:
             out["claim_candidates"], out["claim_shared"] = arr[5], arr[6]
         out["added_spec_pause"] = arr[14]
         out["nfc_spec_pause"], out["nfc_reruns"] = arr[16], arr[17]
         out["merge_pair_wg_per_cu"] = arr[13]
+        out["merge_pair_grid"] = arr[22]
         out["q16_div"] = arr[15]
         out["shortw_slots"], out["shortw_buckets"], out["shortw_max_disp"], out["merge_slots"] = arr[18], arr[19], arr[20], arr[21]
         if arr[12]:
```
